# nixorokish/lodestar

Measured on AMD Instinct MI355X. Metric: BLS signature sets verified/sec (1-8 GPUs) + p50 latency @128-set batch, higher is better.
Workload: dtype u32 (381-bit Fp, 12x32-bit Montgomery limbs); 1 GPU; cfg2: 1024 single-pubkey gossip sets per call, batchable requests, random-scalar batch in chunks of 16 requests; each of the 16 contexts submits 22 calls per pass (bls_gpu_verify_many, one device pass, chunks and verdicts per call); sets_per_call=1024, contexts_per_gpu=16, calls_per_pass=22, calls_in_flight_per_gpu=352, parallelism=shard-by-request x1

## Files before the change

### lodestar_amd/build.py

```python
from __future__ import annotations

import concurrent.futures as cf
import hashlib
import json
import os
import re
import subprocess
import sys
from pathlib import Path

ROOT = Path(__file__).resolve().parent.parent
PKG = ROOT / "lodestar_amd"
CSRC = PKG / "csrc"
OUT_DIR = PKG / "_native"
OBJ_DIR = ROOT / "build" / "obj"
LIB = OUT_DIR / "liblodestar_bls.so"
HIPCC = os.environ.get("HIPCC", "/opt/rocm/bin/hipcc")
ARCH = "gfx950"
FLAGS = ["-O3", "-std=c++17", "-fPIC", f"--offload-arch={ARCH}", "-I", str(ROOT / "include"), "-I", str(CSRC)]


def _headers_digest() -> str:
    h = hashlib.sha256()
    for p in sorted(list(CSRC.rglob("*.hpp")) + list((ROOT / "include").glob("*.h"))):
        h.update(p.name.encode())
        h.update(p.read_bytes())
    return h.hexdigest()


def sources() -> list[Path]:
    return [CSRC / "bls_gpu.hip"] + sorted((CSRC / "kernels").glob("*.hip"))


VARIANTS: dict[str, list[str] | dict[str, list[str]]] = {
}


def _variant_flags(variant: str | None, tu: str) -> list[str] | None:
    if not variant:
        return None
    v = VARIANTS[variant]
    return v if isinstance(v, list) else v.get(tu) or None


ADMISSION_BUDGET = 6 << 30
MIN_QUEUES = 4
SIMDS = 1024


def _resources(remarks: str) -> list[dict]:
    out, cur = [], None
    for line in remarks.splitlines():
        if "remark:" not in line:
            continue
        body = line.split("remark:", 1)[1].strip()
        if body.startswith("Function Name:"):
            cur = {"name": body.split(":", 1)[1].strip().split(" ")[0]}
            out.append(cur)
        elif cur is not None and body.startswith("ScratchSize"):
            cur["scratch"] = int(body.split(":", 1)[1].split()[0])
        elif cur is not None and body.startswith("Occupancy"):
            cur["occupancy"] = int(body.split(":", 1)[1].split()[0])
        elif cur is not None and body.startswith("VGPRs:"):
            cur["vgprs"] = int(body.split(":", 1)[1].split()[0])
        elif cur is not None and body.startswith("AGPRs:"):
            cur["agprs"] = int(body.split(":", 1)[1].split()[0])
    for k in out:
        k["device_scratch_bytes"] = k.get("scratch", 0) * 64 * k.get("occupancy", 1) * SIMDS
    return out


def _check_scratch(src: Path, kernels: list[dict]) -> None:
    cap = ADMISSION_BUDGET // MIN_QUEUES
    for k in kernels:
        if k["device_scratch_bytes"] > cap:
            raise SystemExit(f"{src.name}: kernel {k['name']} reserves {k['device_scratch_bytes'] >> 20} MiB of "
                             f"scratch per queue ({k.get('scratch')} B/lane x 64 x {k.get('occupancy')} waves/SIMD "
                             f"x {SIMDS} SIMDs) > {cap >> 20} MiB: fewer than {MIN_QUEUES} contexts would fit the "
                             "runtime's ~8 GiB (lodestar_amd/build.py ADMISSION_BUDGET)")


FIXTURE_TUS = ("k_sign", "k_probe", "k_peak", "k_selftest", "k_selftest_d28")
FIXTURE_KERNELS = ("k_coop_probe", "k_coop_run_test")


def _plain_name(mangled: str) -> str:
    m = re.match(r"_Z(\d+)", mangled)
    return mangled[m.end(): m.end() + int(m.group(1))] if m else mangled


def scratch_per_queue(table: list[dict]) -> tuple[int, str]:
    path = [k for k in table if k.get("tu") not in FIXTURE_TUS and _plain_name(k["name"]) not in FIXTURE_KERNELS]
    worst = max(path, key=lambda k: k["device_scratch_bytes"])
    fixtures = [k for k in table if k not in path]
    deepest = max(fixtures, key=lambda k: k["device_scratch_bytes"], default=None)
    if deepest is not None and deepest["device_scratch_bytes"] > worst["device_scratch_bytes"]:
        raise RuntimeError(
            f"fixture kernel {_plain_name(deepest['name'])} reserves {deepest['device_scratch_bytes']} B of scratch per "
            f"queue, more than the verify path's deepest ({_plain_name(worst['name'])}, "
            f"{worst['device_scratch_bytes']} B): the admission figure would under-count; shrink it or count it")
    return worst["device_scratch_bytes"], _plain_name(worst["name"])


def _compile(src: Path, hdr: str, verbose: bool, extra: list[str] | None = None) -> Path:
    flags = FLAGS + (extra or [])
    key = hashlib.sha256((hdr + " ".join(flags)).encode() + src.read_bytes()).hexdigest()[:16]
    obj = OBJ_DIR / f"{src.stem}.{key}.o"
    res = obj.with_suffix(".res.json")
    if obj.exists() and res.exists():
        return obj
    cmd = [HIPCC, *flags, "-Rpass-analysis=kernel-resource-usage", "-c", str(src), "-o", str(obj) + ".tmp"]
    if verbose:
        print("[build]", " ".join(cmd), flush=True)
    p = subprocess.run(cmd, capture_output=True, text=True)
    if p.returncode != 0:
        sys.stderr.write(p.stderr)
        raise subprocess.CalledProcessError(p.returncode, cmd)
    kernels = _resources(p.stderr)
    _check_scratch(src, kernels)
    res.write_text(json.dumps(kernels, indent=1))
    os.replace(str(obj) + ".tmp", obj)
    return obj


def build_coop_tables(verbose: bool = True) -> Path:
    tools = ROOT / "tools"
    out = OUT_DIR / "coop_tables.bin"
    gz = OUT_DIR / "coop_tables.bin.gz"
    key = hashlib.sha256(b"".join((tools / f).read_bytes()
                                  for f in ("gen_coop.py", "gen_pset.py", "circuits.py", "gen_constants.py"))).hexdigest()
    stamp = OUT_DIR / ".coop_stamp"
    if gz.exists() and out.with_name("coop_programs.json").exists() and stamp.exists() and stamp.read_text() == key:
        return gz
    if not (out.exists() and stamp.exists() and stamp.read_text() == key):
        if verbose:
            print("[build] tools/gen_coop.py ->", out, flush=True)
        subprocess.run([sys.executable, str(tools / "gen_coop.py"), str(out)], check=True)
    import gzip

    with open(out, "rb") as src, gzip.open(str(gz) + ".tmp", "wb", compresslevel=6) as dst:
        dst.write(src.read())
    os.replace(str(gz) + ".tmp", gz)
    stamp.write_text(key)
    return gz


def build_work_model(verbose: bool = True) -> Path:
    out = OUT_DIR / "work_model.json"
    key = hashlib.sha256(_headers_digest().encode() + (ROOT / "tools" / "work_model.cpp").read_bytes()).hexdigest()
    stamp = OUT_DIR / ".work_stamp"
    if out.exists() and stamp.exists() and stamp.read_text() == key:
        return out
    sys.path.insert(0, str(ROOT / "tools"))
    import work_model

    work_model.build(out, verbose)
    stamp.write_text(key)
    return out


def build(jobs: int | None = None, verbose: bool = True, variant: str | None = None) -> Path:
    OUT_DIR.mkdir(parents=True, exist_ok=True)
    OBJ_DIR.mkdir(parents=True, exist_ok=True)
    build_coop_tables(verbose)
    build_work_model(verbose)
    hdr = _headers_digest()
    srcs = sources()
    lib = OUT_DIR / f"liblodestar_bls_{variant}.so" if variant else LIB
    jobs = jobs or min(len(srcs), os.cpu_count() or 4)
    kern_srcs, host_src = srcs[1:], srcs[0]
    with cf.ThreadPoolExecutor(max_workers=jobs) as ex:
        kobjs = list(ex.map(lambda s: _compile(s, hdr, verbose, _variant_flags(variant, s.stem)), kern_srcs))
    table = [dict(k, tu=o.stem.split(".")[0]) for o in kobjs for k in json.loads(o.with_suffix(".res.json").read_text())]
    per_queue, worst = scratch_per_queue(table)
    host_extra = (_variant_flags(variant, host_src.stem) or []) + [f"-DBLS_SCRATCH_PER_QUEUE={per_queue}ull",
                                                                  f'-DBLS_SCRATCH_WORST_KERNEL="{worst}"']
    objs = [_compile(host_src, hdr, verbose, host_extra)] + kobjs
    if not variant:
        (OUT_DIR / "kernel_resources.json").write_text(json.dumps(
            {"scratch_per_queue": per_queue, "scratch_worst_kernel": worst, "kernels": table}, indent=1))
    stamp = hashlib.sha256("".join(str(o) for o in objs).encode()).hexdigest()
    stamp_file = OUT_DIR / (f".lib_stamp_{variant}" if variant else ".lib_stamp")
    if lib.exists() and stamp_file.exists() and stamp_file.read_text() == stamp:
        return lib
    cmd = [HIPCC, f"--offload-arch={ARCH}", "-shared", "-fPIC", "-o", str(lib) + ".tmp", *map(str, objs), "-lz"]
    if verbose:
        print("[build]", " ".join(cmd), flush=True)
    subprocess.run(cmd, check=True)
    os.replace(str(lib) + ".tmp", lib)
    stamp_file.write_text(stamp)
    return lib


def build_hostsim(verbose: bool = True) -> Path:
    src = ROOT / "tests" / "native" / "hostsim.cpp"
    out = ROOT / "tests" / "native" / "libhostsim.so"
    hdr = _headers_digest()
    key = hashlib.sha256(hdr.encode() + src.read_bytes()).hexdigest()[:16]
    stamp = out.with_suffix(".stamp")
    if out.exists() and stamp.exists() and stamp.read_text() == key:
        return out
    cmd = ["g++", "-O2", "-std=c++17", "-shared", "-fPIC", "-DBLS_COUNT_OPS", "-I", str(CSRC), "-I",
           str(ROOT / "include"), "-o", str(out), str(src)]
    if verbose:
        print("[build]", " ".join(cmd), flush=True)
    subprocess.run(cmd, check=True)
    stamp.write_text(key)
    return out


def build_smsum_host(verbose: bool = True, out: Path | None = None, extra: list[str] | None = None) -> Path:
    src = ROOT / "tests" / "native" / "smsum_host.cpp"
    out = out or ROOT / "tests" / "native" / "smsum_host"
    key = hashlib.sha256((_headers_digest() + " ".join(extra or [])).encode() + src.read_bytes()).hexdigest()[:16]
    stamp = out.with_suffix(".stamp")
    if out.exists() and stamp.exists() and stamp.read_text() == key:
        return out
    cmd = ["g++", "-O2", "-std=c++17", *(extra or []), "-I", str(CSRC), "-I", str(ROOT / "include"), "-o", str(out),
           str(src)]
    if verbose:
        print("[build]", " ".join(cmd), flush=True)
    subprocess.run(cmd, check=True)
    stamp.write_text(key)
    return out


def build_cpu_baseline(verbose: bool = True) -> Path:
    out = ROOT / "oracle" / "cpu" / "libbls_cpu.so"
    cmd = ["make", "-s", "-C", str(ROOT / "oracle" / "cpu")]
    if verbose:
        print("[build]", " ".join(cmd), flush=True)
    subprocess.run(cmd, check=True)
    return out


def build_napi(verbose: bool = True) -> Path | None:
    hdr_dir = Path("/usr/include/node")
    if not (hdr_dir / "node_api.h").exists():
        return None
    src = ROOT / "integration" / "napi" / "lodestar_bls_napi.c"
    out = OUT_DIR / "lodestar_bls.node"
    key = hashlib.sha256(src.read_bytes() + (ROOT / "include" / "lodestar_bls.h").read_bytes()).hexdigest()[:16]
    stamp = OUT_DIR / ".napi_stamp"
    if out.exists() and stamp.exists() and stamp.read_text() == key:
        return out
    cmd = ["gcc", "-O2", "-shared", "-fPIC", "-I", str(hdr_dir), "-I", str(ROOT / "include"), str(src),
           "-L", str(OUT_DIR), "-llodestar_bls", "-Wl,-rpath,$ORIGIN", "-o", str(out)]
    if verbose:
        print("[build]", " ".join(cmd), flush=True)
    subprocess.run(cmd, check=True)
    stamp.write_text(key)
    return out


if __name__ == "__main__":
    if len(sys.argv) > 2 and sys.argv[1] == "--variant":
        build(variant=sys.argv[2])
        sys.exit(0)
    build(jobs=int(sys.argv[1]) if len(sys.argv) > 1 else None)
    build_napi()
    build_hostsim()
    build_smsum_host()
    build_cpu_baseline()
```

### lodestar_amd/csrc/bls/field.hpp

```cpp
#pragma once

#include <stdint.h>
#include <string.h>

#if defined(__HIPCC__)
#include <hip/hip_runtime.h>
#define BLS_HD __host__ __device__ __forceinline__
#define BLS_NOINLINE static __host__ __device__ __attribute__((noinline))
#else
#define BLS_HD static inline
#define BLS_NOINLINE static __attribute__((noinline))
#endif

#if defined(BLS_COUNT_OPS) && !defined(__HIP_DEVICE_COMPILE__)
extern unsigned long long bls_fpm_counter;
#define BLS_COUNT_FPM() (++bls_fpm_counter)
#else
#define BLS_COUNT_FPM() ((void)0)
#endif

namespace bls {

struct Fp {
  uint32_t l[12];
};
struct Fp2 {
  Fp c0, c1;
};
struct Fp6 {
  Fp2 c0, c1, c2;
};
struct Fp12 {
  Fp6 c0, c1;
};

}

#include "constants.hpp"

namespace bls {

BLS_HD uint32_t p_limb(int i) {
  const uint32_t t[12] = {BLS_P_LIMBS};
  return t[i];
}

#if defined(__clang__)
BLS_HD uint32_t addc32(uint32_t a, uint32_t b, uint32_t cin, uint32_t* cout) {
  unsigned co;
  unsigned r = __builtin_addc(a, b, cin, &co);
  *cout = co;
  return r;
}
BLS_HD uint32_t subc32(uint32_t a, uint32_t b, uint32_t bin, uint32_t* bout) {
  unsigned bo;
  unsigned r = __builtin_subc(a, b, bin, &bo);
  *bout = bo;
  return r;
}
#else
BLS_HD uint32_t addc32(uint32_t a, uint32_t b, uint32_t cin, uint32_t* cout) {
  uint64_t t = (uint64_t)a + b + cin;
  *cout = (uint32_t)(t >> 32);
  return (uint32_t)t;
}
BLS_HD uint32_t subc32(uint32_t a, uint32_t b, uint32_t bin, uint32_t* bout) {
  uint64_t t = (uint64_t)a - b - bin;
  *bout = (uint32_t)(t >> 63);
  return (uint32_t)t;
}
#endif

BLS_HD Fp fp_zero() {
  Fp r;
#pragma unroll
  for (int i = 0; i < 12; ++i) r.l[i] = 0;
  return r;
}

BLS_HD bool fp_is_zero(const Fp& a) {
  uint32_t acc = 0;
#pragma unroll
  for (int i = 0; i < 12; ++i) acc |= a.l[i];
  return acc == 0;
}

BLS_HD bool fp_eq(const Fp& a, const Fp& b) {
  uint32_t acc = 0;
#pragma unroll
  for (int i = 0; i < 12; ++i) acc |= a.l[i] ^ b.l[i];
  return acc == 0;
}

BLS_HD Fp fp_select(bool c, const Fp& a, const Fp& b) {
  Fp r;
#pragma unroll
  for (int i = 0; i < 12; ++i) r.l[i] = c ? a.l[i] : b.l[i];
  return r;
}

BLS_HD uint32_t fp_sub_p(const Fp& a, Fp& d) {
  uint32_t borrow = 0;
#pragma unroll
  for (int i = 0; i < 12; ++i) d.l[i] = subc32(a.l[i], p_limb(i), borrow, &borrow);
  return borrow;
}

#if defined(__HIPCC__)
}
#include "carry_asm.hpp"
namespace bls {
#endif

#if defined(__HIP_DEVICE_COMPILE__)
BLS_HD Fp fp_reduce_once(const Fp& s) {
  const uint32_t pl[12] = {BLS_P_LIMBS};
  Fp r;
  asm_reduce12(r.l, s.l, pl);
  return r;
}

BLS_HD Fp fp_add(const Fp& a, const Fp& b) {
  Fp s;
  asm_add12(s.l, a.l, b.l);
  return fp_reduce_once(s);
}

BLS_HD Fp fp_sub(const Fp& a, const Fp& b) {
  const uint32_t pl[12] = {BLS_P_LIMBS};
  Fp d, r;
  uint32_t borrow = asm_sub12(d.l, a.l, b.l);
  asm_add12_masked(r.l, d.l, pl, 0u - borrow);
  return r;
}

BLS_HD Fp fp_add_nr(const Fp& a, const Fp& b) {
  Fp s;
  asm_add12(s.l, a.l, b.l);
  return s;
}

BLS_HD Fp fp_sub_nr(const Fp& a, const Fp& b) {
  const uint32_t pl[12] = {BLS_P_LIMBS};
  Fp t, r;
  (void)asm_sub12(t.l, pl, b.l);
  asm_add12(r.l, a.l, t.l);
  return r;
}

BLS_HD Fp fp_reduce_2p(const Fp& a) {
  const uint32_t pl2[12] = {BLS_2P_LIMBS};
  Fp r;
  asm_reduce12(r.l, a.l, pl2);
  return r;
}
#else
static_assert(sizeof(Fp) == 48, "Fp is 6 x 64-bit words on the host");
static inline void fp_w_load(const Fp& a, uint64_t w[6]) { memcpy(w, a.l, 48); }
static inline Fp fp_w_store(const uint64_t w[6]) {
  Fp r;
  memcpy(r.l, w, 48);
  return r;
}
static const uint64_t BLS_P64[6] = {0xb9feffffffffaaabull, 0x1eabfffeb153ffffull, 0x6730d2a0f6b0f624ull,
                                    0x64774b84f38512bfull, 0x4b1ba7b6434bacd7ull, 0x1a0111ea397fe69aull};
#define BLS_NP0_64 0x89f3fffcfffcfffdull

static inline void fp_w_reduce(uint64_t s[6]) {
  uint64_t d[6];
  unsigned __int128 br = 0;
  for (int i = 0; i < 6; ++i) {
    const unsigned __int128 t = (unsigned __int128)s[i] - BLS_P64[i] - (uint64_t)br;
    d[i] = (uint64_t)t;
    br = (t >> 64) & 1;
  }
  if (!br) memcpy(s, d, 48);
}

BLS_HD Fp fp_reduce_once(const Fp& a) {
  uint64_t s[6];
  fp_w_load(a, s);
  fp_w_reduce(s);
  return fp_w_store(s);
}

BLS_HD Fp fp_add(const Fp& a, const Fp& b) {
  uint64_t x[6], y[6];
  fp_w_load(a, x);
  fp_w_load(b, y);
  unsigned __int128 c = 0;
  for (int i = 0; i < 6; ++i) {
    c += (unsigned __int128)x[i] + y[i];
    x[i] = (uint64_t)c;
    c >>= 64;
  }
  fp_w_reduce(x);
  return fp_w_store(x);
}

BLS_HD Fp fp_sub(const Fp& a, const Fp& b) {
  uint64_t x[6], y[6];
  fp_w_load(a, x);
  fp_w_load(b, y);
  unsigned __int128 br = 0;
  for (int i = 0; i < 6; ++i) {
    const unsigned __int128 t = (unsigned __int128)x[i] - y[i] - (uint64_t)br;
    x[i] = (uint64_t)t;
    br = (t >> 64) & 1;
  }
  if (br) {
    unsigned __int128 c = 0;
    for (int i = 0; i < 6; ++i) {
      c += (unsigned __int128)x[i] + BLS_P64[i];
      x[i] = (uint64_t)c;
      c >>= 64;
    }
  }
  return fp_w_store(x);
}

BLS_HD Fp fp_add_nr(const Fp& a, const Fp& b) {
  uint64_t x[6], y[6];
  fp_w_load(a, x);
  fp_w_load(b, y);
  unsigned __int128 c = 0;
  for (int i = 0; i < 6; ++i) {
    c += (unsigned __int128)x[i] + y[i];
    x[i] = (uint64_t)c;
    c >>= 64;
  }
  return fp_w_store(x);
}

BLS_HD Fp fp_sub_nr(const Fp& a, const Fp& b) {
  uint64_t x[6], y[6];
  fp_w_load(a, x);
  fp_w_load(b, y);
  unsigned __int128 br = 0, c = 0;
  for (int i = 0; i < 6; ++i) {
    const unsigned __int128 t = (unsigned __int128)BLS_P64[i] - y[i] - (uint64_t)br;
    y[i] = (uint64_t)t;
    br = (t >> 64) & 1;
  }
  for (int i = 0; i < 6; ++i) {
    c += (unsigned __int128)x[i] + y[i];
    x[i] = (uint64_t)c;
    c >>= 64;
  }
  return fp_w_store(x);
}

BLS_HD Fp fp_reduce_2p(const Fp& a) {
  static const uint64_t P2[6] = {0x73fdffffffff5556ull, 0x3d57fffd62a7ffffull, 0xce61a541ed61ec48ull,
                                 0xc8ee9709e70a257eull, 0x96374f6c869759aeull, 0x340223d472ffcd34ull};
  uint64_t x[6], d[6];
  fp_w_load(a, x);
  unsigned __int128 br = 0;
  for (int i = 0; i < 6; ++i) {
    const unsigned __int128 t = (unsigned __int128)x[i] - P2[i] - (uint64_t)br;
    d[i] = (uint64_t)t;
    br = (t >> 64) & 1;
  }
  return fp_w_store(br ? x : d);
}
#endif

BLS_HD Fp fp_dbl(const Fp& a) { return fp_add(a, a); }

BLS_HD Fp fp_neg(const Fp& a) {
  Fp z = fp_zero();
  return fp_sub(z, a);
}

BLS_HD Fp fp_half(const Fp& a) {
  uint32_t mask = 0u - (a.l[0] & 1u);
  Fp s;
  uint32_t c = 0;
#pragma unroll
  for (int i = 0; i < 12; ++i) s.l[i] = addc32(a.l[i], p_limb(i) & mask, c, &c);
  Fp r;
#pragma unroll
  for (int i = 0; i < 11; ++i) r.l[i] = (s.l[i] >> 1) | (s.l[i + 1] << 31);
  r.l[11] = s.l[11] >> 1;
  return r;
}

#define BLS_D28_MASK 0xFFFFFFFu
#define BLS_NP28 0xFFCFFFDu
BLS_HD uint32_t p28_digit(int k) {
  const uint32_t t[14] = {0xfffaaabu, 0xfefffffu, 0x3ffffb9u, 0xfffeb15u, 0x6241eabu, 0xa0f6b0fu, 0xf6730d2u,
                          0xf38512bu, 0x4774b84u, 0x4bacd76u, 0xba7b643u, 0xe69a4b1u, 0x1ea397fu, 0x001a011u};
  return t[k];
}

BLS_HD void fp_to_d28(const Fp& a, uint32_t d[14]) {
#pragma unroll
  for (int k = 0; k < 14; ++k) {
    const int o = 28 * k, w = o >> 5, s = o & 31;
    const uint64_t pair = ((uint64_t)(w + 1 < 12 ? a.l[w + 1] : 0u) << 32) | a.l[w];
    d[k] = (uint32_t)(pair >> s) & BLS_D28_MASK;
  }
}

#if defined(__HIP_DEVICE_COMPILE__)
#define BLS_D28_MAC(t, a, b)                                                        \
  do {                                                                              \
    uint64_t cc_;                                                                   \
    asm volatile("v_mad_u64_u32 %0, %1, %2, %3, %0" : "+v"(t), "=&s"(cc_) : "v"(a), "v"(b)); \
  } while (0)
#define BLS_D28_MACS(t, a, b)                                                       \
  do {                                                                              \
    uint64_t cc_;                                                                   \
    asm volatile("v_mad_i64_i32 %0, %1, %2, %3, %0" : "+v"(t), "=&s"(cc_) : "v"(a), "v"(b)); \
  } while (0)
#define BLS_PIN_FP(c)                                                                                \
  asm volatile("" ::"v"((c).l[0]), "v"((c).l[1]), "v"((c).l[2]), "v"((c).l[3]), "v"((c).l[4]),     \
               "v"((c).l[5]), "v"((c).l[6]), "v"((c).l[7]), "v"((c).l[8]), "v"((c).l[9]), "v"((c).l[10]), \
               "v"((c).l[11]))
#define BLS_D28_MACK(t, a, k)                                                                        \
  do {                                                                                               \
    uint64_t cc_;                                                                                    \
    asm volatile("v_mad_u64_u32 %0, %1, %2, %3, %0" : "+v"(t), "=&s"(cc_) : "v"(a), "s"(k));        \
  } while (0)
#else
#define BLS_D28_MACK(t, a, k) ((t) += (uint64_t)(a) * (k))
#define BLS_PIN_FP(c) ((void)0)
#define BLS_D28_MAC(t, a, b) ((t) += (uint64_t)(a) * (b))
#define BLS_D28_MACS(t, a, b) ((t) = (uint64_t)((int64_t)(t) + (int64_t)(int32_t)(a) * (int64_t)(int32_t)(b)))
#endif

BLS_HD Fp fp_d28_tail(uint64_t t[27]);

template <bool ORDERED = false>
BLS_HD Fp fp_redc_d28(uint64_t t[27]) {
#pragma unroll
  for (int i = 0; i < 13; ++i) {
    const uint32_t m = ((uint32_t)t[i] * BLS_NP28) & BLS_D28_MASK;
#pragma unroll
    for (int j = 0; j < 14; ++j) {
      if (ORDERED) BLS_D28_MACK(t[i + j], m, p28_digit(j));
      else t[i + j] += (uint64_t)m * p28_digit(j);
    }
    t[i + 1] += t[i] >> 28;
  }
  {
    const uint32_t m = ((uint32_t)t[13] * BLS_NP28) & 0xFFFFFu;
#pragma unroll
    for (int j = 0; j < 14; ++j) {
      if (ORDERED) BLS_D28_MACK(t[13 + j], m, p28_digit(j));
      else t[13 + j] += (uint64_t)m * p28_digit(j);
    }
  }
  return fp_d28_tail(t);
}

BLS_HD Fp fp_d28_tail(uint64_t t[27]) {
  const uint64_t u = t[13] >> 20;
  t[14] += u >> 8;
#pragma unroll
  for (int k = 14; k < 26; ++k) {
    t[k + 1] += t[k] >> 28;
    t[k] &= BLS_D28_MASK;
  }
  Fp r;
  uint64_t acc = u & 0xFFu;
  int nb = 8, w = 0;
#pragma unroll
  for (int k = 14; k < 27; ++k) {
    acc |= t[k] << nb;
    nb += 28;
    while (nb >= 32 && w < 12) {
      r.l[w++] = (uint32_t)acc;
      acc >>= 32;
      nb -= 32;
    }
  }
  while (w < 12) {
    r.l[w++] = (uint32_t)acc;
    acc >>= 32;
  }
  return r;
}

BLS_HD Fp fp_mul_d28_lazy(const Fp& a, const Fp& b) {
  uint32_t x[14], y[14];
  fp_to_d28(a, x);
  fp_to_d28(b, y);
  uint64_t t[27];
#pragma unroll
  for (int k = 0; k < 27; ++k) t[k] = 0;
#pragma unroll
  for (int i = 0; i < 14; ++i)
#pragma unroll
    for (int j = 0; j < 14; ++j) t[i + j] += (uint64_t)x[i] * y[j];
  return fp_redc_d28(t);
}

BLS_HD Fp fp_sqr_d28_lazy(const Fp& a) {
  uint32_t x[14], x2[14];
  fp_to_d28(a, x);
#pragma unroll
  for (int k = 0; k < 14; ++k) x2[k] = x[k] << 1;
  uint64_t t[27];
#pragma unroll
  for (int k = 0; k < 27; ++k) t[k] = 0;
#pragma unroll
  for (int i = 0; i < 14; ++i) {
    t[2 * i] += (uint64_t)x[i] * x[i];
#pragma unroll
    for (int j = i + 1; j < 14; ++j) t[i + j] += (uint64_t)x2[i] * x[j];
  }
  return fp_redc_d28(t);
}

BLS_HD uint64_t c2_col(int k) {
  const uint64_t t[27] = {
      0x00ffffffe1cc48ddull, 0x01ffffffcec8d82dull, 0x02ffffffa9e42d7cull, 0x03ffffff8c5f88ffull, 0x04ffffff683c5c79ull,
      0x05ffffff4a84a061ull, 0x06ffffff2f404920ull, 0x07ffffff0efefe3bull, 0x08fffffee90b358cull, 0x09fffffec66cc7e1ull,
      0x0afffffea7af04abull, 0x0bfffffe892c9c2eull, 0x0cfffffe6149107bull, 0x0c0034009ffe581bull, 0x0b003400bffcbfe9ull,
      0x0a003400dffcbfe8ull, 0x09003400fffcbfe7ull, 0x080034011ffcbfe6ull, 0x070034013ffcbfe5ull, 0x060034015ffcbfe4ull,
      0x050034017ffcbfe3ull, 0x040034019ffcbfe2ull, 0x03003401bffcbfe1ull, 0x02003401dffcbfe0ull, 0x01003401fffcbfdfull,
      0x000034021ffcbfdeull, 0x00000002a4374121ull};
  return t[k];
}

#if defined(__HIP_DEVICE_COMPILE__)
#define BLS_SCHED_FENCE() __builtin_amdgcn_sched_barrier(0)
#else
#define BLS_SCHED_FENCE() ((void)0)
#endif

BLS_HD Fp2 fp2_mul_d28(const Fp& a0, const Fp& a1, const Fp& b0, const Fp& b1) {
  uint32_t x0[14], x1[14], y0[14], y1[14];
  fp_to_d28(a0, x0);
  fp_to_d28(a1, x1);
  fp_to_d28(b0, y0);
  fp_to_d28(b1, y1);
  uint64_t t[27];
  int32_t ny1[14];
#pragma unroll
  for (int j = 0; j < 14; ++j) ny1[j] = -(int32_t)y1[j];
#pragma unroll
  for (int k = 0; k < 27; ++k) t[k] = c2_col(k);
#pragma unroll
  for (int i = 0; i < 14; ++i)
#pragma unroll
    for (int j = 0; j < 14; ++j) {
      BLS_D28_MAC(t[i + j], x0[i], y0[j]);
      BLS_D28_MACS(t[i + j], x1[i], ny1[j]);
    }
  const Fp c0 = fp_reduce_once(fp_redc_d28<true>(t));
  BLS_PIN_FP(c0);
  BLS_SCHED_FENCE();
#pragma unroll
  for (int k = 0; k < 27; ++k) t[k] = 0;
#pragma unroll
  for (int i = 0; i < 14; ++i)
#pragma unroll
    for (int j = 0; j < 14; ++j) {
      BLS_D28_MAC(t[i + j], x0[i], y1[j]);
      BLS_D28_MAC(t[i + j], x1[i], y0[j]);
    }
  return Fp2{c0, fp_reduce_once(fp_redc_d28<true>(t))};
}

BLS_HD Fp2 fp2_sqr_d28(const Fp& a0, const Fp& a1) {
  uint32_t x0[14], x1[14];
  fp_to_d28(a0, x0);
  fp_to_d28(a1, x1);
  uint64_t t[27];
  int32_t n1[14], n2[14];
#pragma unroll
  for (int j = 0; j < 14; ++j) {
    n1[j] = -(int32_t)x1[j];
    n2[j] = -(int32_t)(x1[j] << 1);
  }
#pragma unroll
  for (int k = 0; k < 27; ++k) t[k] = c2_col(k);
#pragma unroll
  for (int i = 0; i < 14; ++i) {
    BLS_D28_MAC(t[2 * i], x0[i], x0[i]);
    BLS_D28_MACS(t[2 * i], x1[i], n1[i]);
#pragma unroll
    for (int j = i + 1; j < 14; ++j) {
      BLS_D28_MAC(t[i + j], x0[i] << 1, x0[j]);
      BLS_D28_MACS(t[i + j], x1[i], n2[j]);
    }
  }
  const Fp c0 = fp_reduce_once(fp_redc_d28<true>(t));
  BLS_PIN_FP(c0);
  BLS_SCHED_FENCE();
#pragma unroll
  for (int k = 0; k < 27; ++k) t[k] = 0;
#pragma unroll
  for (int i = 0; i < 14; ++i)
#pragma unroll
    for (int j = 0; j < 14; ++j) BLS_D28_MAC(t[i + j], x0[i] << 1, x1[j]);
  return Fp2{c0, fp_reduce_once(fp_redc_d28<true>(t))};
}

#if defined(__HIP_DEVICE_COMPILE__)
__device__ __forceinline__ void bls_mac(uint64_t& lo, uint32_t& hi, uint32_t a, uint32_t b) {
  uint64_t cc;
  asm("v_mad_u64_u32 %0, %2, %3, %4, %0\n\t"
      "v_addc_co_u32 %1, %2, 0, %1, %2"
      : "+v"(lo), "+v"(hi), "=&s"(cc)
      : "v"(a), "v"(b));
}
__device__ __forceinline__ void bls_mac_s(uint64_t& lo, uint32_t& hi, uint32_t a, uint32_t b) {
  uint64_t cc;
  asm("v_mad_u64_u32 %0, %2, %3, %4, %0\n\t"
      "v_addc_co_u32 %1, %2, 0, %1, %2"
      : "+v"(lo), "+v"(hi), "=&s"(cc)
      : "v"(a), "s"(b));
}
__device__ __forceinline__ void bls_mac2(uint64_t& lo, uint32_t& hi, uint32_t a, uint32_t b, uint64_t& lo2,
                                         uint32_t& hi2, uint32_t m, uint32_t p) {
  uint64_t c1, c2;
  asm("v_mad_u64_u32 %0, %4, %6, %7, %0\n\t"
      "v_mad_u64_u32 %2, %5, %8, %9, %2\n\t"
      "v_addc_co_u32 %1, %4, 0, %1, %4\n\t"
      "v_addc_co_u32 %3, %5, 0, %3, %5"
      : "+v"(lo), "+v"(hi), "+v"(lo2), "+v"(hi2), "=&s"(c1), "=&s"(c2)
      : "v"(a), "v"(b), "v"(m), "s"(p));
}

#define BLS_MAC4(L, H, k, x, y0, y1, y2, y3, YC)                                                       \
  do {                                                                                             \
    uint64_t c0_, c1_, c2_, c3_;                                                                   \
    asm("v_mad_u64_u32 %0, %8, %12, %13, %0\n\t"                                                  \
        "v_mad_u64_u32 %2, %9, %12, %14, %2\n\t"                                                  \
        "v_mad_u64_u32 %4, %10, %12, %15, %4\n\t"                                                 \
        "v_mad_u64_u32 %6, %11, %12, %16, %6\n\t"                                                 \
        "v_addc_co_u32 %1, %8, 0, %1, %8\n\t"                                                     \
        "v_addc_co_u32 %3, %9, 0, %3, %9\n\t"                                                     \
        "v_addc_co_u32 %5, %10, 0, %5, %10\n\t"                                                   \
        "v_addc_co_u32 %7, %11, 0, %7, %11"                                                        \
        : "+v"(L[k]), "+v"(H[k]), "+v"(L[k + 1]), "+v"(H[k + 1]), "+v"(L[k + 2]), "+v"(H[k + 2]),   \
          "+v"(L[k + 3]), "+v"(H[k + 3]), "=&s"(c0_), "=&s"(c1_), "=&s"(c2_), "=&s"(c3_)            \
        : "v"(x), YC(y0), YC(y1), YC(y2), YC(y3));                                                  \
  } while (0)

__device__ __forceinline__ void bls_col_add(uint64_t& lo, uint32_t& hi, uint64_t c) {
  uint32_t l0 = (uint32_t)lo, l1 = (uint32_t)(lo >> 32);
  uint64_t cc;
  asm("v_add_co_u32 %0, %3, %0, %4\n\t"
      "v_addc_co_u32 %1, %3, %1, %5, %3\n\t"
      "v_addc_co_u32 %2, %3, 0, %2, %3"
      : "+v"(l0), "+v"(l1), "+v"(hi), "=&s"(cc)
      : "v"((uint32_t)c), "v"((uint32_t)(c >> 32)));
  lo = ((uint64_t)l1 << 32) | l0;
}

template <bool LAZY>
__device__ __forceinline__ Fp fp_mul_cols(const Fp& a, const Fp& b) {
  uint64_t L[24];
  uint32_t H[24];
#pragma unroll
  for (int k = 0; k < 24; ++k) {
    L[k] = 0;
    H[k] = 0;
  }
#pragma unroll
  for (int i = 0; i < 12; ++i) {
#pragma unroll
    for (int j = 0; j < 12; j += 4) BLS_MAC4(L, H, i + j, a.l[i], b.l[j], b.l[j + 1], b.l[j + 2], b.l[j + 3], "v");
  }
#pragma unroll
  for (int i = 0; i < 12; ++i) {
    const uint32_t m = (uint32_t)L[i] * BLS_NP0;
    BLS_MAC4(L, H, i, m, p_limb(0), p_limb(1), p_limb(2), p_limb(3), "s");
    const uint64_t c = (L[i] >> 32) | ((uint64_t)H[i] << 32);
    bls_col_add(L[i + 1], H[i + 1], c);
    BLS_MAC4(L, H, i + 4, m, p_limb(4), p_limb(5), p_limb(6), p_limb(7), "s");
    BLS_MAC4(L, H, i + 8, m, p_limb(8), p_limb(9), p_limb(10), p_limb(11), "s");
  }
  Fp u;
#pragma unroll
  for (int k = 12; k < 23; ++k) {
    u.l[k - 12] = (uint32_t)L[k];
    const uint64_t c = (L[k] >> 32) | ((uint64_t)H[k] << 32);
    bls_col_add(L[k + 1], H[k + 1], c);
  }
  u.l[11] = (uint32_t)L[23];
  return LAZY ? u : fp_reduce_once(u);
}
__device__ __forceinline__ Fp fp_sqr_cols(const Fp& a) {
  uint64_t L[24];
  uint32_t H[24];
#pragma unroll
  for (int k = 0; k < 24; ++k) {
    L[k] = 0;
    H[k] = 0;
  }
#pragma unroll
  for (int i = 0; i < 11; ++i) {
    int j = i + 1;
#pragma unroll
    for (; j + 3 < 12; j += 4) BLS_MAC4(L, H, i + j, a.l[i], a.l[j], a.l[j + 1], a.l[j + 2], a.l[j + 3], "v");
#pragma unroll
    for (; j < 12; ++j) bls_mac(L[i + j], H[i + j], a.l[i], a.l[j]);
  }
#pragma unroll
  for (int k = 1; k < 23; ++k) {
    H[k] = (H[k] << 1) | (uint32_t)(L[k] >> 63);
    L[k] <<= 1;
  }
#pragma unroll
  for (int i = 0; i < 12; ++i) bls_mac(L[2 * i], H[2 * i], a.l[i], a.l[i]);
#pragma unroll
  for (int i = 0; i < 12; ++i) {
    const uint32_t m = (uint32_t)L[i] * BLS_NP0;
    BLS_MAC4(L, H, i, m, p_limb(0), p_limb(1), p_limb(2), p_limb(3), "s");
    const uint64_t c = (L[i] >> 32) | ((uint64_t)H[i] << 32);
    bls_col_add(L[i + 1], H[i + 1], c);
    BLS_MAC4(L, H, i + 4, m, p_limb(4), p_limb(5), p_limb(6), p_limb(7), "s");
    BLS_MAC4(L, H, i + 8, m, p_limb(8), p_limb(9), p_limb(10), p_limb(11), "s");
  }
  Fp u;
#pragma unroll
  for (int k = 12; k < 23; ++k) {
    u.l[k - 12] = (uint32_t)L[k];
    const uint64_t c = (L[k] >> 32) | ((uint64_t)H[k] << 32);
    bls_col_add(L[k + 1], H[k + 1], c);
  }
  u.l[11] = (uint32_t)L[23];
  return fp_reduce_once(u);
}
#ifdef BLS_FP_INLINE
#define BLS_FP_MUL_ATTR static __device__ __forceinline__
#else
#define BLS_FP_MUL_ATTR BLS_NOINLINE
#endif
#if !defined(BLS_FP_D28)
BLS_FP_MUL_ATTR Fp fp_sqr_dev(Fp a) { return fp_sqr_cols(a); }
__device__ __forceinline__ Fp fp_mul_inl(const Fp& a, const Fp& b) { return fp_mul_cols<false>(a, b); }
__device__ __forceinline__ Fp fp_mul_lazy(const Fp& a, const Fp& b) { return fp_mul_cols<true>(a, b); }
#else
BLS_FP_MUL_ATTR Fp fp_sqr_dev(Fp a) { return fp_reduce_once(fp_sqr_d28_lazy(a)); }
__device__ __forceinline__ Fp fp_mul_inl(const Fp& a, const Fp& b) { return fp_reduce_once(fp_mul_d28_lazy(a, b)); }
__device__ __forceinline__ Fp fp_mul_lazy(const Fp& a, const Fp& b) { return fp_mul_d28_lazy(a, b); }
#endif
#define BLS_W12(x) uint32_t x##0, uint32_t x##1, uint32_t x##2, uint32_t x##3, uint32_t x##4, uint32_t x##5, \
                   uint32_t x##6, uint32_t x##7, uint32_t x##8, uint32_t x##9, uint32_t x##10, uint32_t x##11
#define BLS_FP_OF(x) Fp{{x##0, x##1, x##2, x##3, x##4, x##5, x##6, x##7, x##8, x##9, x##10, x##11}}
#define BLS_L12(v) (v).l[0], (v).l[1], (v).l[2], (v).l[3], (v).l[4], (v).l[5], (v).l[6], (v).l[7], (v).l[8], \
                   (v).l[9], (v).l[10], (v).l[11]
BLS_FP_MUL_ATTR Fp fp_mul_w(BLS_W12(a), BLS_W12(b)) { return fp_mul_inl(BLS_FP_OF(a), BLS_FP_OF(b)); }
BLS_FP_MUL_ATTR Fp fp_sqr_w(BLS_W12(a)) { return fp_sqr_dev(BLS_FP_OF(a)); }
__device__ __forceinline__ Fp fp_mul(const Fp& a, const Fp& b) { return fp_mul_w(BLS_L12(a), BLS_L12(b)); }
#else
BLS_HD Fp fp_mul(const Fp& a, const Fp& b) {
  BLS_COUNT_FPM();
  typedef unsigned __int128 u128;
  uint64_t x[6], y[6], t[13];
  fp_w_load(a, x);
  fp_w_load(b, y);
  for (int k = 0; k < 13; ++k) t[k] = 0;
  for (int i = 0; i < 6; ++i) {
    uint64_t c = 0;
    for (int j = 0; j < 6; ++j) {
      const u128 v = (u128)x[i] * y[j] + t[i + j] + c;
      t[i + j] = (uint64_t)v;
      c = (uint64_t)(v >> 64);
    }
    t[i + 6] = c;
  }
  for (int i = 0; i < 6; ++i) {
    const uint64_t m = t[i] * BLS_NP0_64;
    uint64_t c = 0;
    for (int j = 0; j < 6; ++j) {
      const u128 v = (u128)m * BLS_P64[j] + t[i + j] + c;
      t[i + j] = (uint64_t)v;
      c = (uint64_t)(v >> 64);
    }
    for (int k = i + 6; k < 13 && c; ++k) {
      const u128 v = (u128)t[k] + c;
      t[k] = (uint64_t)v;
      c = (uint64_t)(v >> 64);
    }
  }
  fp_w_reduce(t + 6);
  return fp_w_store(t + 6);
}
BLS_HD Fp fp_mul_inl(const Fp& a, const Fp& b) { return fp_mul(a, b); }
BLS_HD Fp fp_mul_lazy(const Fp& a, const Fp& b) { return fp_mul(a, b); }
#endif

#if defined(__HIP_DEVICE_COMPILE__)
BLS_HD Fp fp_sqr(const Fp& a) { return fp_sqr_w(BLS_L12(a)); }
#else
BLS_HD Fp fp_sqr(const Fp& a) { return fp_mul(a, a); }
#endif

BLS_HD Fp fp_to_mont(const Fp& a) { return fp_mul(a, c_r2()); }

BLS_HD Fp fp_from_mont(const Fp& a) {
  Fp one = fp_zero();
  one.l[0] = 1;
  return fp_mul(a, one);
}

}
#include "lazy28.hpp"
namespace bls {

#if defined(__HIP_DEVICE_COMPILE__) && !defined(BLS_LAZY_POW)
#define BLS_LAZY_POW 1
#endif
#ifdef BLS_LAZY_POW
template <uint32_t (*E)(int), int BITS>
BLS_HD Fp fp_pow_const(const Fp& a) {
  return lz_pow_const<E, BITS>(a);
}
#else
template <uint32_t (*E)(int), int BITS>
BLS_HD Fp fp_pow_const(const Fp& a) {
  Fp tab[8];
  tab[0] = a;
  const Fp a2 = fp_sqr(a);
  for (int k = 1; k < 8; ++k) tab[k] = fp_mul(tab[k - 1], a2);
  Fp r = a;
  bool started = false;
  int i = BITS - 1;
  while (i >= 0) {
    if (!((E(i >> 5) >> (i & 31)) & 1u)) {
      r = fp_sqr(r);
      --i;
      continue;
    }
    int j = i - 3 < 0 ? 0 : i - 3;
    while (!((E(j >> 5) >> (j & 31)) & 1u)) ++j;
    uint32_t val = 0;
    for (int k = i; k >= j; --k) {
      val = (val << 1) | ((E(k >> 5) >> (k & 31)) & 1u);
      if (started) r = fp_sqr(r);
    }
    r = started ? fp_mul(r, tab[val >> 1]) : tab[val >> 1];
    started = true;
    i = j - 1;
  }
  return r;
}
#endif

BLS_HD Fp fp_inv(const Fp& a) { return fp_pow_const<e_p_minus_2, E_P_MINUS_2_BITS>(a); }

BLS_HD bool big_is_one(const Fp& a) {
  uint32_t acc = a.l[0] ^ 1u;
#pragma unroll
  for (int i = 1; i < 12; ++i) acc |= a.l[i];
  return acc == 0;
}

BLS_HD void big_shr1(Fp& a) {
#pragma unroll
  for (int i = 0; i < 11; ++i) a.l[i] = (a.l[i] >> 1) | (a.l[i + 1] << 31);
  a.l[11] >>= 1;
}

BLS_HD bool big_geq(const Fp& a, const Fp& b) {
  uint32_t borrow = 0;
#pragma unroll
  for (int i = 0; i < 12; ++i) {
    uint64_t t = (uint64_t)a.l[i] - b.l[i] - borrow;
    borrow = (uint32_t)(t >> 63);
  }
  return borrow == 0;
}

BLS_HD void big_sub(Fp& a, const Fp& b) {
  uint32_t borrow = 0;
#pragma unroll
  for (int i = 0; i < 12; ++i) {
    uint64_t t = (uint64_t)a.l[i] - b.l[i] - borrow;
    a.l[i] = (uint32_t)t;
    borrow = (uint32_t)(t >> 63);
  }
}

struct Big13 {
  uint32_t l[13];
};

BLS_HD Big13 big13_lin_shr30(const Big13& x, const Big13& y, int32_t u, int32_t v) {
  uint32_t t[13];
  int64_t carry = 0;
#pragma unroll
  for (int i = 0; i < 13; ++i) {
    const int64_t xi = i < 12 ? (int64_t)x.l[i] : (int64_t)(int32_t)x.l[i];
    const int64_t yi = i < 12 ? (int64_t)y.l[i] : (int64_t)(int32_t)y.l[i];
    const int64_t s = carry + (int64_t)u * xi + (int64_t)v * yi;
    t[i] = (uint32_t)s;
    carry = s >> 32;
  }
  Big13 r;
#pragma unroll
  for (int i = 0; i < 12; ++i) r.l[i] = (t[i] >> 30) | (t[i + 1] << 2);
  r.l[12] = (uint32_t)((int32_t)t[12] >> 30);
  return r;
}

BLS_HD Big13 big13_lin_modp_shr30(const Big13& d, const Big13& e, int32_t u, int32_t v) {
  uint32_t t[13];
  int64_t carry = 0;
#pragma unroll
  for (int i = 0; i < 13; ++i) {
    const int64_t di = i < 12 ? (int64_t)d.l[i] : (int64_t)(int32_t)d.l[i];
    const int64_t ei = i < 12 ? (int64_t)e.l[i] : (int64_t)(int32_t)e.l[i];
    const int64_t s = carry + (int64_t)u * di + (int64_t)v * ei;
    t[i] = (uint32_t)s;
    carry = s >> 32;
  }
  const uint32_t k = (t[0] * BLS_NP0) & 0x3fffffffu;
  uint64_t c = 0;
#pragma unroll
  for (int i = 0; i < 12; ++i) {
    const uint64_t s = (uint64_t)t[i] + (uint64_t)k * p_limb(i) + c;
    t[i] = (uint32_t)s;
    c = s >> 32;
  }
  t[12] += (uint32_t)c;
  Big13 r;
#pragma unroll
  for (int i = 0; i < 12; ++i) r.l[i] = (t[i] >> 30) | (t[i + 1] << 2);
  r.l[12] = (uint32_t)((int32_t)t[12] >> 30);
  Big13 m;
  uint32_t borrow = 0;
#pragma unroll
  for (int i = 0; i < 13; ++i) {
    const uint64_t s = (uint64_t)r.l[i] - (i < 12 ? p_limb(i) : 0u) - borrow;
    m.l[i] = (uint32_t)s;
    borrow = (uint32_t)(s >> 63);
  }
  const bool ge_p = (int32_t)m.l[12] >= 0;
  uint32_t cc = 0;
  Big13 q;
#pragma unroll
  for (int i = 0; i < 13; ++i) {
    const uint64_t s = (uint64_t)r.l[i] + (i < 12 ? p_limb(i) : 0u) + cc;
    q.l[i] = (uint32_t)s;
    cc = (uint32_t)(s >> 32);
  }
  const bool lt_mp = (int32_t)q.l[12] < 0;
#pragma unroll
  for (int i = 0; i < 13; ++i) r.l[i] = ge_p ? m.l[i] : (lt_mp ? q.l[i] : r.l[i]);
  return r;
}

BLS_NOINLINE Fp fp_inv_gcd(Fp a) {
  if (fp_is_zero(a)) return fp_zero();
  Big13 f, g, d, e;
#pragma unroll
  for (int i = 0; i < 12; ++i) {
    f.l[i] = p_limb(i);
    g.l[i] = a.l[i];
    d.l[i] = 0;
    e.l[i] = 0;
  }
  f.l[12] = g.l[12] = d.l[12] = e.l[12] = 0;
  e.l[0] = 1;
  int32_t delta = 1;
  for (int round = 0; round < 37; ++round) {
    uint32_t fl = f.l[0], gl = g.l[0];
    int32_t u = 1, v = 0, q = 0, r = 1;
    for (int s = 0; s < 30; ++s) {
      const bool godd = (gl & 1u) != 0;
      const bool swap = godd && delta > 0;
      const uint32_t nfl = swap ? gl : fl, ngl = swap ? (0u - fl) : gl;
      const int32_t nu = swap ? q : u, nv = swap ? r : v, nq = swap ? -u : q, nr = swap ? -v : r;
      delta = swap ? -delta : delta;
      fl = nfl;
      gl = ngl;
      u = nu;
      v = nv;
      q = nq;
      r = nr;
      gl += godd ? fl : 0u;
      q += godd ? u : 0;
      r += godd ? v : 0;
      gl >>= 1;
      u *= 2;
      v *= 2;
      delta += 1;
    }
    const Big13 f2 = big13_lin_shr30(f, g, u, v);
    const Big13 g2 = big13_lin_shr30(f, g, q, r);
    const Big13 d2 = big13_lin_modp_shr30(d, e, u, v);
    const Big13 e2 = big13_lin_modp_shr30(d, e, q, r);
    f = f2;
    g = g2;
    d = d2;
    e = e2;
  }
  const bool fneg = (int32_t)f.l[12] < 0;
  Big13 x;
  uint32_t borrow = 0;
#pragma unroll
  for (int i = 0; i < 13; ++i) {
    const uint64_t s = (uint64_t)0 - d.l[i] - borrow;
    x.l[i] = fneg ? (uint32_t)s : d.l[i];
    borrow = (uint32_t)(s >> 63);
  }
  const bool xneg = (int32_t)x.l[12] < 0;
  Fp inv;
  uint32_t c = 0;
#pragma unroll
  for (int i = 0; i < 12; ++i) {
    const uint64_t s = (uint64_t)x.l[i] + (xneg ? p_limb(i) : 0u) + c;
    inv.l[i] = (uint32_t)s;
    c = (uint32_t)(s >> 32);
  }
  return fp_mul(inv, c_r3());
}


BLS_HD bool fp_plain_gt_half(const Fp& a) {
  const uint32_t h[12] = {BLS_HALF_P_LIMBS};
  uint32_t borrow = 0;
#pragma unroll
  for (int i = 0; i < 12; ++i) {
    uint64_t t = (uint64_t)h[i] - a.l[i] - borrow;
    borrow = (uint32_t)(t >> 63);
  }
  return borrow != 0;
}

BLS_HD bool fp_lex_largest(const Fp& a_mont) { return fp_plain_gt_half(fp_from_mont(a_mont)); }

BLS_HD bool fp_plain_is_canonical(const Fp& a) {
  Fp d;
  return fp_sub_p(a, d) != 0;
}

BLS_HD Fp fp_from_be48(const uint8_t* b) {
  Fp r;
#pragma unroll
  for (int k = 0; k < 12; ++k) {
    const uint8_t* q = b + 44 - 4 * k;
    r.l[k] = ((uint32_t)q[0] << 24) | ((uint32_t)q[1] << 16) | ((uint32_t)q[2] << 8) | (uint32_t)q[3];
  }
  return r;
}

BLS_HD void fp_to_be48(const Fp& a, uint8_t* b) {
#pragma unroll
  for (int k = 0; k < 12; ++k) {
    uint8_t* q = b + 44 - 4 * k;
    q[0] = (uint8_t)(a.l[k] >> 24);
    q[1] = (uint8_t)(a.l[k] >> 16);
    q[2] = (uint8_t)(a.l[k] >> 8);
    q[3] = (uint8_t)a.l[k];
  }
}

BLS_HD bool fp_sqrt(const Fp& a, Fp& r) {
  r = fp_pow_const<e_p_plus_1_div_4, E_P_PLUS_1_DIV_4_BITS>(a);
  return fp_eq(fp_sqr(r), a);
}

BLS_HD Fp2 fp2_zero() { return Fp2{fp_zero(), fp_zero()}; }
BLS_HD Fp2 fp2_one() { return Fp2{c_one(), fp_zero()}; }
BLS_HD bool fp2_is_zero(const Fp2& a) { return fp_is_zero(a.c0) && fp_is_zero(a.c1); }
BLS_HD bool fp2_eq(const Fp2& a, const Fp2& b) { return fp_eq(a.c0, b.c0) && fp_eq(a.c1, b.c1); }
BLS_HD Fp2 fp2_select(bool c, const Fp2& a, const Fp2& b) {
  return Fp2{fp_select(c, a.c0, b.c0), fp_select(c, a.c1, b.c1)};
}
BLS_HD Fp2 fp2_add(const Fp2& a, const Fp2& b) { return Fp2{fp_add(a.c0, b.c0), fp_add(a.c1, b.c1)}; }
BLS_HD Fp2 fp2_sub(const Fp2& a, const Fp2& b) { return Fp2{fp_sub(a.c0, b.c0), fp_sub(a.c1, b.c1)}; }
BLS_HD Fp2 fp2_dbl(const Fp2& a) { return Fp2{fp_dbl(a.c0), fp_dbl(a.c1)}; }
BLS_HD Fp2 fp2_neg(const Fp2& a) { return Fp2{fp_neg(a.c0), fp_neg(a.c1)}; }
BLS_HD Fp2 fp2_conj(const Fp2& a) { return Fp2{a.c0, fp_neg(a.c1)}; }
BLS_HD Fp2 fp2_half(const Fp2& a) { return Fp2{fp_half(a.c0), fp_half(a.c1)}; }
BLS_HD Fp2 fp2_mul_fp(const Fp2& a, const Fp& b) { return Fp2{fp_mul(a.c0, b), fp_mul(a.c1, b)}; }

BLS_HD Fp2 fp2_mul(const Fp2& a, const Fp2& b) {
  Fp t0 = fp_mul(a.c0, b.c0);
  Fp t1 = fp_mul(a.c1, b.c1);
  Fp t2 = fp_mul(fp_add_nr(a.c0, a.c1), fp_add_nr(b.c0, b.c1));
  return Fp2{fp_sub(t0, t1), fp_sub(fp_sub(t2, t0), t1)};
}

BLS_HD Fp2 fp2_mul_s(const Fp2& a, const Fp2& b) {
  Fp t0 = fp_mul(a.c0, b.c0);
  Fp t1 = fp_mul(a.c1, b.c1);
  Fp t2 = fp_mul(fp_reduce_2p(fp_add_nr(a.c0, a.c1)), fp_add_nr(b.c0, b.c1));
  return Fp2{fp_sub(t0, t1), fp_sub(fp_sub(t2, t0), t1)};
}
BLS_HD Fp2 fp2_add_nr(const Fp2& a, const Fp2& b) { return Fp2{fp_add_nr(a.c0, b.c0), fp_add_nr(a.c1, b.c1)}; }

BLS_HD Fp2 fp2_sqr(const Fp2& a) {
  Fp t0 = fp_mul(fp_add_nr(a.c0, a.c1), fp_sub_nr(a.c0, a.c1));
  Fp t1 = fp_mul(fp_add_nr(a.c0, a.c0), a.c1);
  return Fp2{t0, t1};
}

BLS_HD Fp2 fp2_mul_xi(const Fp2& a) { return Fp2{fp_sub(a.c0, a.c1), fp_add(a.c0, a.c1)}; }

BLS_HD Fp2 fp2_inv(const Fp2& a) {
  Fp n = fp_add(fp_sqr(a.c0), fp_sqr(a.c1));
  Fp ni = fp_inv(n);
  return Fp2{fp_mul(a.c0, ni), fp_neg(fp_mul(a.c1, ni))};
}

BLS_HD uint32_t fp2_sgn0(const Fp2& a) {
  Fp p0 = fp_from_mont(a.c0);
  Fp p1 = fp_from_mont(a.c1);
  uint32_t s0 = p0.l[0] & 1u;
  uint32_t z0 = fp_is_zero(p0) ? 1u : 0u;
  uint32_t s1 = p1.l[0] & 1u;
  return s0 | (z0 & s1);
}

BLS_HD bool fp2_lex_largest(const Fp2& a) {
  Fp p1 = fp_from_mont(a.c1);
  if (!fp_is_zero(p1)) return fp_plain_gt_half(p1);
  return fp_plain_gt_half(fp_from_mont(a.c0));
}

BLS_HD bool fp2_sqrt(const Fp2& a, Fp2& r) {
  if (fp_is_zero(a.c1)) {
    Fp s;
    if (fp_sqrt(a.c0, s)) {
      r = Fp2{s, fp_zero()};
      return true;
    }
    fp_sqrt(fp_neg(a.c0), s);
    r = Fp2{fp_zero(), s};
    return true;
  }
  Fp alpha = fp_add(fp_sqr(a.c0), fp_sqr(a.c1));
  Fp gamma;
  if (!fp_sqrt(alpha, gamma)) return false;
  Fp d = fp_half(fp_add(a.c0, gamma));
  Fp t = fp_pow_const<e_p_minus_3_div_4, E_P_MINUS_3_DIV_4_BITS>(d);
  Fp dt = fp_mul(d, t);
  Fp a1t2 = fp_half(fp_mul(a.c1, t));
  if (fp_eq(fp_sqr(dt), d)) {
    r = Fp2{dt, a1t2};
  } else {
    r = Fp2{a1t2, fp_neg(dt)};
  }
  return true;
}

BLS_HD Fp6 fp6_zero() { return Fp6{fp2_zero(), fp2_zero(), fp2_zero()}; }
BLS_HD Fp6 fp6_one() { return Fp6{fp2_one(), fp2_zero(), fp2_zero()}; }
BLS_HD Fp6 fp6_add(const Fp6& a, const Fp6& b) {
  return Fp6{fp2_add(a.c0, b.c0), fp2_add(a.c1, b.c1), fp2_add(a.c2, b.c2)};
}
BLS_HD Fp6 fp6_sub(const Fp6& a, const Fp6& b) {
  return Fp6{fp2_sub(a.c0, b.c0), fp2_sub(a.c1, b.c1), fp2_sub(a.c2, b.c2)};
}
BLS_HD Fp6 fp6_neg(const Fp6& a) { return Fp6{fp2_neg(a.c0), fp2_neg(a.c1), fp2_neg(a.c2)}; }
BLS_HD bool fp6_eq(const Fp6& a, const Fp6& b) {
  return fp2_eq(a.c0, b.c0) && fp2_eq(a.c1, b.c1) && fp2_eq(a.c2, b.c2);
}
BLS_HD Fp6 fp6_mul_v(const Fp6& a) { return Fp6{fp2_mul_xi(a.c2), a.c0, a.c1}; }

BLS_HD Fp6 fp6_mul(const Fp6& a, const Fp6& b) {
  Fp2 t0 = fp2_mul(a.c0, b.c0);
  Fp2 t1 = fp2_mul(a.c1, b.c1);
  Fp2 t2 = fp2_mul(a.c2, b.c2);
  Fp2 c0 = fp2_sub(fp2_sub(fp2_mul_s(fp2_add_nr(a.c1, a.c2), fp2_add_nr(b.c1, b.c2)), t1), t2);
  c0 = fp2_add(fp2_mul_xi(c0), t0);
  Fp2 c1 = fp2_sub(fp2_sub(fp2_mul_s(fp2_add_nr(a.c0, a.c1), fp2_add_nr(b.c0, b.c1)), t0), t1);
  c1 = fp2_add(c1, fp2_mul_xi(t2));
  Fp2 c2 = fp2_sub(fp2_sub(fp2_mul_s(fp2_add_nr(a.c0, a.c2), fp2_add_nr(b.c0, b.c2)), t0), t2);
  c2 = fp2_add(c2, t1);
  return Fp6{c0, c1, c2};
}

BLS_HD Fp6 fp6_sqr(const Fp6& a) { return fp6_mul(a, a); }

BLS_HD Fp6 fp6_mul_01(const Fp6& a, const Fp2& d0, const Fp2& d1) {
  Fp2 a0d0 = fp2_mul(a.c0, d0);
  Fp2 a1d1 = fp2_mul(a.c1, d1);
  Fp2 c0 = fp2_add(a0d0, fp2_mul_xi(fp2_mul(a.c2, d1)));
  Fp2 c1 = fp2_sub(fp2_sub(fp2_mul_s(fp2_add_nr(a.c0, a.c1), fp2_add_nr(d0, d1)), a0d0), a1d1);
  Fp2 c2 = fp2_add(a1d1, fp2_mul(a.c2, d0));
  return Fp6{c0, c1, c2};
}

BLS_HD Fp6 fp6_mul_1(const Fp6& a, const Fp2& d1) {
  return Fp6{fp2_mul_xi(fp2_mul(a.c2, d1)), fp2_mul(a.c0, d1), fp2_mul(a.c1, d1)};
}

BLS_HD Fp6 fp6_inv(const Fp6& a) {
  Fp2 t0 = fp2_sub(fp2_sqr(a.c0), fp2_mul_xi(fp2_mul(a.c1, a.c2)));
  Fp2 t1 = fp2_sub(fp2_mul_xi(fp2_sqr(a.c2)), fp2_mul(a.c0, a.c1));
  Fp2 t2 = fp2_sub(fp2_sqr(a.c1), fp2_mul(a.c0, a.c2));
  Fp2 n = fp2_add(fp2_mul(a.c0, t0), fp2_mul_xi(fp2_add(fp2_mul(a.c2, t1), fp2_mul(a.c1, t2))));
  Fp2 ni = fp2_inv(n);
  return Fp6{fp2_mul(t0, ni), fp2_mul(t1, ni), fp2_mul(t2, ni)};
}

BLS_HD Fp12 fp12_one() { return Fp12{fp6_one(), fp6_zero()}; }
BLS_HD bool fp12_eq(const Fp12& a, const Fp12& b) { return fp6_eq(a.c0, b.c0) && fp6_eq(a.c1, b.c1); }
BLS_HD bool fp12_is_one(const Fp12& a) { return fp12_eq(a, fp12_one()); }
BLS_HD Fp12 fp12_conj(const Fp12& a) { return Fp12{a.c0, fp6_neg(a.c1)}; }

BLS_NOINLINE Fp12 fp12_mul(const Fp12& a, const Fp12& b) {
  Fp6 t0 = fp6_mul(a.c0, b.c0);
  Fp6 t1 = fp6_mul(a.c1, b.c1);
  Fp6 c1 = fp6_sub(fp6_sub(fp6_mul(fp6_add(a.c0, a.c1), fp6_add(b.c0, b.c1)), t0), t1);
  Fp6 c0 = fp6_add(t0, fp6_mul_v(t1));
  return Fp12{c0, c1};
}

BLS_NOINLINE Fp12 fp12_sqr(const Fp12& a) {
  Fp6 ab = fp6_mul(a.c0, a.c1);
  Fp6 s = fp6_mul(fp6_add(a.c0, a.c1), fp6_add(a.c0, fp6_mul_v(a.c1)));
  Fp6 c0 = fp6_sub(fp6_sub(s, ab), fp6_mul_v(ab));
  Fp6 c1 = fp6_add(ab, ab);
  return Fp12{c0, c1};
}

BLS_NOINLINE Fp12 fp12_mul_line(const Fp12& f, const Fp2& l0, const Fp2& l2, const Fp2& l3) {
  Fp6 aa = fp6_mul_01(f.c0, l0, l2);
  Fp6 bb = fp6_mul_1(f.c1, l3);
  Fp6 c1 = fp6_sub(fp6_sub(fp6_mul_01(fp6_add(f.c0, f.c1), l0, fp2_add(l2, l3)), aa), bb);
  Fp6 c0 = fp6_add(aa, fp6_mul_v(bb));
  return Fp12{c0, c1};
}

BLS_HD Fp12 fp12_mul_line2(const Fp12& f, const Fp2& l0, const Fp2& l2, const Fp2& l3, const Fp2& m0,
                           const Fp2& m2, const Fp2& m3) {
  const Fp2 m00 = fp2_mul(l0, m0), m22 = fp2_mul(l2, m2), m33 = fp2_mul(l3, m3);
  const Fp2 a0 = fp2_add(m00, fp2_mul_xi(m33));
  const Fp2 a2 = fp2_sub(fp2_sub(fp2_mul_s(fp2_add_nr(l0, l2), fp2_add_nr(m0, m2)), m00), m22);
  const Fp2 a3 = fp2_sub(fp2_sub(fp2_mul_s(fp2_add_nr(l0, l3), fp2_add_nr(m0, m3)), m00), m33);
  const Fp2 a5 = fp2_sub(fp2_sub(fp2_mul_s(fp2_add_nr(l2, l3), fp2_add_nr(m2, m3)), m22), m33);
  const Fp6 p0 = Fp6{a0, a2, m22};
  const Fp6 t0 = fp6_mul(f.c0, p0);
  const Fp6 t1 = fp6_mul_v(fp6_mul_01(f.c1, a3, a5));
  const Fp6 c1 = fp6_sub(fp6_sub(fp6_mul(fp6_add(f.c0, f.c1), Fp6{a0, fp2_add(a2, a3), fp2_add(m22, a5)}), t0), t1);
  return Fp12{fp6_add(t0, fp6_mul_v(t1)), c1};
}

BLS_HD Fp6 fp12_sqr_half_prod(const Fp12& a, bool h) {
  return fp6_mul(h ? fp6_add(a.c0, a.c1) : a.c0, h ? fp6_add(a.c0, fp6_mul_v(a.c1)) : a.c1);
}
BLS_HD Fp12 fp12_sqr_half_join(const Fp6& own, const Fp6& other, bool h) {
  const Fp6 ab = h ? other : own, s = h ? own : other;
  return Fp12{fp6_sub(fp6_sub(s, ab), fp6_mul_v(ab)), fp6_add(ab, ab)};
}
struct LineHalf {
  Fp6 m;
  Fp2 p, q;
};
BLS_HD LineHalf fp12_line_half_prod(const Fp12& f, const Fp2& l0, const Fp2& l2, const Fp2& l3, bool h) {
  LineHalf r;
  r.m = fp6_mul_01(h ? fp6_add(f.c0, f.c1) : f.c0, l0, h ? fp2_add(l2, l3) : l2);
  r.p = fp2_mul(h ? f.c1.c0 : f.c1.c2, l3);
  r.q = fp2_mul(f.c1.c1, l3);
  return r;
}
BLS_HD Fp12 fp12_line_half_join(const LineHalf& own, const Fp6& m_other, const Fp2& p_other, bool h) {
  const Fp6 aa = h ? m_other : own.m, t = h ? own.m : m_other;
  const Fp6 bb = Fp6{fp2_mul_xi(h ? p_other : own.p), h ? own.p : p_other, own.q};
  return Fp12{fp6_add(aa, fp6_mul_v(bb)), fp6_sub(fp6_sub(t, aa), bb)};
}

BLS_HD Fp12 fp12_inv(const Fp12& a) {
  Fp6 n = fp6_sub(fp6_sqr(a.c0), fp6_mul_v(fp6_sqr(a.c1)));
  Fp6 ni = fp6_inv(n);
  return Fp12{fp6_mul(a.c0, ni), fp6_neg(fp6_mul(a.c1, ni))};
}

BLS_HD Fp12 fp12_frob(const Fp12& a) {
  Fp12 r;
  r.c0.c0 = fp2_conj(a.c0.c0);
  r.c1.c0 = fp2_mul(fp2_conj(a.c1.c0), c_frob1_1());
  r.c0.c1 = fp2_mul(fp2_conj(a.c0.c1), c_frob1_2());
  r.c1.c1 = fp2_mul(fp2_conj(a.c1.c1), c_frob1_3());
  r.c0.c2 = fp2_mul(fp2_conj(a.c0.c2), c_frob1_4());
  r.c1.c2 = fp2_mul(fp2_conj(a.c1.c2), c_frob1_5());
  return r;
}

BLS_HD Fp12 fp12_frob2(const Fp12& a) {
  Fp12 r;
  r.c0.c0 = a.c0.c0;
  r.c1.c0 = fp2_mul_fp(a.c1.c0, c_frob2_1());
  r.c0.c1 = fp2_mul_fp(a.c0.c1, c_frob2_2());
  r.c1.c1 = fp2_mul_fp(a.c1.c1, c_frob2_3());
  r.c0.c2 = fp2_mul_fp(a.c0.c2, c_frob2_4());
  r.c1.c2 = fp2_mul_fp(a.c1.c2, c_frob2_5());
  return r;
}

BLS_HD void fp4_sqr(const Fp2& x, const Fp2& y, Fp2& rx, Fp2& ry) {
  Fp2 t0 = fp2_sqr(x);
  Fp2 t1 = fp2_sqr(y);
  rx = fp2_add(t0, fp2_mul_xi(t1));
  ry = fp2_sub(fp2_sub(fp2_sqr(fp2_add(x, y)), t0), t1);
}

BLS_NOINLINE Fp12 fp12_cyclotomic_sqr(const Fp12& f) {
  Fp2 a0, a1, b0, b1, d0, d1;
  fp4_sqr(f.c0.c0, f.c1.c1, a0, a1);
  fp4_sqr(f.c1.c0, f.c0.c2, b0, b1);
  fp4_sqr(f.c0.c1, f.c1.c2, d0, d1);
  Fp12 r;
  r.c0.c0 = fp2_add(fp2_dbl(fp2_sub(a0, f.c0.c0)), a0);
  r.c1.c1 = fp2_add(fp2_dbl(fp2_add(a1, f.c1.c1)), a1);
  Fp2 xd1 = fp2_mul_xi(d1);
  r.c1.c0 = fp2_add(fp2_dbl(fp2_add(xd1, f.c1.c0)), xd1);
  r.c0.c2 = fp2_add(fp2_dbl(fp2_sub(d0, f.c0.c2)), d0);
  r.c0.c1 = fp2_add(fp2_dbl(fp2_sub(b0, f.c0.c1)), b0);
  r.c1.c2 = fp2_add(fp2_dbl(fp2_add(b1, f.c1.c2)), b1);
  return r;
}

}
```

### lodestar_amd/csrc/kernels/field_ops.hpp

```cpp
#pragma once

#include "../launchers.hpp"
#include "../bls/selftest_ops.hpp"

namespace bls {

enum : uint32_t {
  FOP_ADD = 0,
  FOP_SUB,
  FOP_NEG,
  FOP_DBL,
  FOP_HALF,
  FOP_ADD_NR,
  FOP_SUB_NR,
  FOP_REDUCE_ONCE,
  FOP_REDUCE_2P,
  FOP_CANON3,
  FOP_MUL,
  FOP_SQR,
  FOP_MUL_LAZY,
  FOP_SQR_D28_LAZY,
  FOP_FP2_MUL_D28,
  FOP_FP2_SQR_D28,
  FOP_FP2_MUL,
  FOP_FP2_SQR,
  FOP_FP2_MUL_S,
  FOP_LZ_MUL_RAW,
  FOP_LZ_SQR_RAW,
  FOP_LZ_FP_OPS,
  FOP_LZ_FP2_OPS,
  FOP_INV,
  FOP_INV_GCD,
  FOP_SQRT,
  FOP_FP2_INV,
  FOP_FP2_SQRT,
  FOP_LIN8,
  FOP_COUNT
};
#define FOP_D28_FLAG 0x100u
#define FOP_LIN8_IN 102

constexpr int field_op_in_words(uint32_t op) {
  return op == FOP_NEG || op == FOP_DBL || op == FOP_HALF || op == FOP_REDUCE_ONCE || op == FOP_REDUCE_2P ||
                 op == FOP_CANON3 || op == FOP_SQR || op == FOP_SQR_D28_LAZY || op == FOP_INV ||
                 op == FOP_INV_GCD || op == FOP_SQRT
             ? 12
         : op == FOP_FP2_MUL_D28 || op == FOP_FP2_MUL || op == FOP_FP2_MUL_S || op == FOP_LZ_FP2_OPS ? 48
         : op == FOP_LZ_MUL_RAW                                                                        ? 28
         : op == FOP_LZ_SQR_RAW                                                                        ? 14
         : op == FOP_LIN8                                                                              ? FOP_LIN8_IN
                                                                                                       : 24;
}
constexpr int field_op_out_words(uint32_t op) {
  return op == FOP_FP2_MUL_D28 || op == FOP_FP2_SQR_D28 || op == FOP_FP2_MUL || op == FOP_FP2_SQR ||
                 op == FOP_FP2_MUL_S || op == FOP_FP2_INV
             ? 24
         : op == FOP_LZ_MUL_RAW || op == FOP_LZ_SQR_RAW ? 14
         : op == FOP_LZ_FP_OPS                          ? 120
         : op == FOP_LZ_FP2_OPS                         ? 144
         : op == FOP_SQRT                               ? 13
         : op == FOP_FP2_SQRT                           ? 25
                                                        : 12;
}

constexpr bool field_op_d28_only(uint32_t op) { return op == FOP_CANON3 || op >= FOP_SQR_D28_LAZY; }

#if defined(BLS_FP_D28)
#define FOP_IS_D28 true
#else
#define FOP_IS_D28 false
#endif

__device__ __forceinline__ Fp fop_ld(const uint32_t* w, int k) {
  Fp r;
#pragma unroll
  for (int i = 0; i < 12; ++i) r.l[i] = w[12 * k + i];
  return r;
}
__device__ __forceinline__ void fop_st(uint32_t* w, int k, const Fp& v) {
#pragma unroll
  for (int i = 0; i < 12; ++i) w[12 * k + i] = v.l[i];
}
__device__ __forceinline__ Fp2 fop_ld2(const uint32_t* w, int k) { return Fp2{fop_ld(w, 2 * k), fop_ld(w, 2 * k + 1)}; }
__device__ __forceinline__ void fop_st2(uint32_t* w, int k, const Fp2& v) {
  fop_st(w, 2 * k, v.c0);
  fop_st(w, 2 * k + 1, v.c1);
}

template <uint32_t OP, bool D28>
__device__ __forceinline__ void field_op_body(const uint32_t* x, uint32_t* y) {
  if constexpr (OP == FOP_ADD) fop_st(y, 0, fp_add(fop_ld(x, 0), fop_ld(x, 1)));
  else if constexpr (OP == FOP_SUB) fop_st(y, 0, fp_sub(fop_ld(x, 0), fop_ld(x, 1)));
  else if constexpr (OP == FOP_NEG) fop_st(y, 0, fp_neg(fop_ld(x, 0)));
  else if constexpr (OP == FOP_DBL) fop_st(y, 0, fp_dbl(fop_ld(x, 0)));
  else if constexpr (OP == FOP_HALF) fop_st(y, 0, fp_half(fop_ld(x, 0)));
  else if constexpr (OP == FOP_ADD_NR) fop_st(y, 0, fp_add_nr(fop_ld(x, 0), fop_ld(x, 1)));
  else if constexpr (OP == FOP_SUB_NR) fop_st(y, 0, fp_sub_nr(fop_ld(x, 0), fop_ld(x, 1)));
  else if constexpr (OP == FOP_REDUCE_ONCE) fop_st(y, 0, fp_reduce_once(fop_ld(x, 0)));
  else if constexpr (OP == FOP_REDUCE_2P) fop_st(y, 0, fp_reduce_2p(fop_ld(x, 0)));
  else if constexpr (OP == FOP_CANON3) fop_st(y, 0, fp_canon3(fop_ld(x, 0)));
  else if constexpr (OP == FOP_MUL) fop_st(y, 0, fp_mul(fop_ld(x, 0), fop_ld(x, 1)));
  else if constexpr (OP == FOP_SQR) fop_st(y, 0, fp_sqr(fop_ld(x, 0)));
  else if constexpr (OP == FOP_MUL_LAZY) fop_st(y, 0, fp_mul_lazy(fop_ld(x, 0), fop_ld(x, 1)));
#if defined(BLS_FP_D28)
  else if constexpr (OP == FOP_SQR_D28_LAZY) fop_st(y, 0, fp_sqr_d28_lazy(fop_ld(x, 0)));
  else if constexpr (OP == FOP_FP2_MUL_D28)
    fop_st2(y, 0, fp2_mul_d28(fop_ld(x, 0), fop_ld(x, 1), fop_ld(x, 2), fop_ld(x, 3)));
  else if constexpr (OP == FOP_FP2_SQR_D28) fop_st2(y, 0, fp2_sqr_d28(fop_ld(x, 0), fop_ld(x, 1)));
  else if constexpr (OP == FOP_FP2_MUL) fop_st2(y, 0, fp2_mul(fop_ld2(x, 0), fop_ld2(x, 1)));
  else if constexpr (OP == FOP_FP2_SQR) fop_st2(y, 0, fp2_sqr(fop_ld2(x, 0)));
  else if constexpr (OP == FOP_FP2_MUL_S) fop_st2(y, 0, fp2_mul_s(fop_ld2(x, 0), fop_ld2(x, 1)));
  else if constexpr (OP == FOP_LZ_MUL_RAW || OP == FOP_LZ_SQR_RAW) {
    Lz14 a, b;
#pragma unroll
    for (int k = 0; k < 14; ++k) {
      a.d[k] = (int32_t)x[k];
      b.d[k] = OP == FOP_LZ_MUL_RAW ? (int32_t)x[14 + k] : 0;
    }
    const Lz14 r = OP == FOP_LZ_MUL_RAW ? lz_mul_w(LZ_L14(a), LZ_L14(b)) : lz_sqr_w(LZ_L14(a));
#pragma unroll
    for (int k = 0; k < 14; ++k) y[k] = (uint32_t)r.d[k];
  } else if constexpr (OP == FOP_LZ_FP_OPS) {
    Fp r[10];
    sf_lz_fp_ops(fop_ld(x, 0), fop_ld(x, 1), r);
    for (int k = 0; k < 10; ++k) fop_st(y, k, r[k]);
  } else if constexpr (OP == FOP_LZ_FP2_OPS) {
    Fp2 r[6];
    sf_lz_fp2_ops(fop_ld2(x, 0), fop_ld2(x, 1), r);
    for (int k = 0; k < 6; ++k) fop_st2(y, k, r[k]);
  } else if constexpr (OP == FOP_INV) fop_st(y, 0, fp_inv(fop_ld(x, 0)));
  else if constexpr (OP == FOP_INV_GCD) fop_st(y, 0, fp_inv_gcd(fop_ld(x, 0)));
  else if constexpr (OP == FOP_SQRT) {
    Fp r = fp_zero();
    y[0] = fp_sqrt(fop_ld(x, 0), r) ? 1u : 0u;
    fop_st(y + 1, 0, r);
  } else if constexpr (OP == FOP_FP2_INV) fop_st2(y, 0, fp2_inv(fop_ld2(x, 0)));
  else if constexpr (OP == FOP_FP2_SQRT) {
    Fp2 r = fp2_zero();
    y[0] = fp2_sqrt(fop_ld2(x, 0), r) ? 1u : 0u;
    fop_st2(y + 1, 0, r);
  }
#endif
}

template <uint32_t OP, bool D28, int IN, int OUT>
__global__ __launch_bounds__(BLS_BLOCK) void k_field_op(const uint32_t* __restrict__ in, uint32_t n,
                                                        uint32_t* __restrict__ out) {
  const uint32_t i = blockIdx.x * BLS_BLOCK + threadIdx.x;
  if (i >= n) return;
  uint32_t x[IN], y[OUT];
#pragma unroll
  for (int k = 0; k < IN; ++k) x[k] = in[(size_t)IN * i + k];
#pragma unroll
  for (int k = 0; k < OUT; ++k) y[k] = 0;
  field_op_body<OP, D28>(x, y);
#pragma unroll
  for (int k = 0; k < OUT; ++k) out[(size_t)OUT * i + k] = y[k];
}

#if defined(BLS_FP_D28)
template <bool D28>
__global__ __launch_bounds__(BLS_BLOCK) void k_field_lin8(const uint32_t* __restrict__ in, uint32_t n,
                                                          uint32_t* __restrict__ out) {
  __shared__ Fp vals[BLS_BLOCK * 8];
  __shared__ int s_nmax;
  const uint32_t lane = threadIdx.x, i = blockIdx.x * BLS_BLOCK + lane;
  const bool live = i < n;
  if (lane == 0) s_nmax = 0;
  __syncthreads();
  uint16_t refs[8];
  int16_t cf[8];
#pragma unroll
  for (int k = 0; k < 8; ++k) {
    refs[k] = 0;
    cf[k] = 0;
  }
  int nt = 0;
  bool single = false;
  if (live) {
    const uint32_t* rec = in + (size_t)FOP_LIN8_IN * i;
    nt = rec[100] < 8u ? (int)rec[100] : 8;
    single = (rec[101] & 1u) != 0;
#pragma unroll
    for (int k = 0; k < 8; ++k) {
      lds_store_fp(vals, lane * 8 + k, fop_ld(rec, k));
      if (k < nt) {
        refs[k] = (uint16_t)(lane * 8 + k);
        cf[k] = (int16_t)(rec[96 + (k >> 1)] >> (16 * (k & 1)));
      }
    }
    atomicMax(&s_nmax, nt);
  }
  __syncthreads();
  const int nmax = __builtin_amdgcn_readfirstlane(s_nmax);
  const Fp r = coop_lin(refs, cf, nt, nmax, single, (const LdsU4*)vals);
  if (live) fop_st(out + 12ull * i, 0, r);
}
#endif

#define FOP_CASE(OP)                                                                                    \
  case OP:                                                                                              \
    k_field_op<OP, FOP_IS_D28, field_op_in_words(OP), field_op_out_words(OP)>                            \
        <<<bls_grid_for(n), BLS_BLOCK, 0, s>>>(in, n, out);                                             \
    break

static hipError_t field_op_launch(uint32_t op, const uint32_t* in, uint32_t n, uint32_t* out, hipStream_t s) {
  switch (op) {
    FOP_CASE(FOP_ADD);
    FOP_CASE(FOP_SUB);
    FOP_CASE(FOP_NEG);
    FOP_CASE(FOP_DBL);
    FOP_CASE(FOP_HALF);
    FOP_CASE(FOP_ADD_NR);
    FOP_CASE(FOP_SUB_NR);
    FOP_CASE(FOP_REDUCE_ONCE);
    FOP_CASE(FOP_REDUCE_2P);
    FOP_CASE(FOP_MUL);
    FOP_CASE(FOP_SQR);
    FOP_CASE(FOP_MUL_LAZY);
#if defined(BLS_FP_D28)
    FOP_CASE(FOP_CANON3);
    FOP_CASE(FOP_SQR_D28_LAZY);
    FOP_CASE(FOP_FP2_MUL_D28);
    FOP_CASE(FOP_FP2_SQR_D28);
    FOP_CASE(FOP_FP2_MUL);
    FOP_CASE(FOP_FP2_SQR);
    FOP_CASE(FOP_FP2_MUL_S);
    FOP_CASE(FOP_LZ_MUL_RAW);
    FOP_CASE(FOP_LZ_SQR_RAW);
    FOP_CASE(FOP_LZ_FP_OPS);
    FOP_CASE(FOP_LZ_FP2_OPS);
    FOP_CASE(FOP_INV);
    FOP_CASE(FOP_INV_GCD);
    FOP_CASE(FOP_SQRT);
    FOP_CASE(FOP_FP2_INV);
    FOP_CASE(FOP_FP2_SQRT);
    case FOP_LIN8:
      k_field_lin8<true><<<bls_grid_for(n), BLS_BLOCK, 0, s>>>(in, n, out);
      break;
#endif
    default:
      return hipErrorInvalidValue;
  }
  return hipGetLastError();
}

}
```

### lodestar_amd/csrc/kernels/k_chain.hip

```cpp
#define BLS_FP_D28 1
#include "../launchers.hpp"

using namespace bls;

namespace {

__device__ __noinline__ void iso_jac_nl(G2J* out, const Fp* q) { *out = iso_map_jac(Fp2{q[0], q[1]}, Fp2{q[2], q[3]}); }

__device__ __noinline__ void g2_mul_aff(G2J* out, const G2A* in, uint64_t k) { *out = aff_mul_u64(*in, k); }
__device__ __noinline__ void g2_mul_r(G2J* out, const G2A* in, uint64_t k, G2J* T) {
  uint32_t a, b;
  glv_split(k, a, b);
  *out = in->inf ? jac_infinity<Fp2>() : jac_mul_glv<Fp2>(jac_from_aff(*in), a, b, T);
}
__device__ __noinline__ void g1_mul_r(G1J* out, const G1J* in, uint64_t k, G1J* T) {
  uint32_t a, b;
  glv_split(k, a, b);
  *out = jac_mul_glv<Fp>(*in, a, b, T);
}
__device__ __noinline__ void g2_add(G2J* out, const G2J* a, const G2J* b) { *out = jac_add(*a, *b); }

__device__ __noinline__ void g2_to_aff(G2A* out, const G2J* in) {
  if (jac_is_inf(*in)) {
    out->x = fp2_zero();
    out->y = fp2_zero();
    out->inf = true;
    return;
  }
  const Fp ni = fp_inv_gcd(fp_add(fp_sqr(in->z.c0), fp_sqr(in->z.c1)));
  const Fp2 zi = Fp2{fp_mul(in->z.c0, ni), fp_neg(fp_mul(in->z.c1, ni))};
  const Fp2 zi2 = fp2_sqr(zi);
  out->x = fp2_mul(in->x, zi2);
  out->y = fp2_mul(in->y, fp2_mul(zi2, zi));
  out->inf = false;
}

__device__ __noinline__ void g2_mul_x_aff(G2J* out, const G2J* p) {
  G2A a;
  g2_to_aff(&a, p);
  g2_mul_aff(out, &a, (uint64_t)BLS_X_ABS);
  out->y = fp2_neg(out->y);
}

__device__ void store_one(Fp12* f) {
  Fp* d = reinterpret_cast<Fp*>(f);
  d[0] = c_one();
#pragma unroll
  for (int k = 1; k < 12; ++k) d[k] = fp_zero();
}

__device__ void flag_exact(const PipeBufs& b, uint32_t i) {
  b.set_flag[i] = 1u;
  atomicAdd(b.flag_count, 1u);
}

}

__device__ bool chain_skip(const PipeBufs& b, uint32_t i) {
  return b.pk_status[i] != BLS_OK || b.sig_status[i] != BLS_OK || jac_is_inf(b.pk[i]) || b.sig[i].inf ||
         b.set_flag[i];
}

__device__ __noinline__ void chain_role_h(Fp* chain, const Fp* qs, uint8_t* chain_st, uint32_t i) {
  Fp* o = chain + (size_t)CHAIN_WORDS * i;
  const Fp* q = qs + 8ull * i;
  G2J A, B, C;
  iso_jac_nl(&A, q);
  iso_jac_nl(&B, q + 4);
  g2_add(&A, &A, &B);
  g2_mul_x_aff(&B, &A);
  C = g2_psi(A);
  g2_add(&B, &B, &C);
  C = g2_psi(g2_psi(jac_dbl(A)));
  g2_add(&A, &B, &A);
  A.y = fp2_neg(A.y);
  g2_add(&C, &C, &A);
  g2_mul_x_aff(&A, &B);
  g2_add(&A, &A, &C);
  chain_st[4 * i + 0] = jac_is_inf(A) ? 1 : 0;
  if (jac_is_inf(A)) return;
  const Fp ni = fp_inv_gcd(fp_add(fp_sqr(A.z.c0), fp_sqr(A.z.c1)));
  const Fp2 zi = Fp2{fp_mul(A.z.c0, ni), fp_neg(fp_mul(A.z.c1, ni))};
  const Fp2 zi2 = fp2_sqr(zi);
  const Fp2 hx = fp2_mul(A.x, zi2);
  const Fp2 hy = fp2_mul(A.y, fp2_mul(zi2, zi));
  o[CH_HQ + 0] = hx.c0;
  o[CH_HQ + 1] = hx.c1;
  o[CH_HQ + 2] = hy.c0;
  o[CH_HQ + 3] = hy.c1;
}

__device__ __noinline__ void chain_role_sub(const G2A* sigs, uint8_t* chain_st, uint32_t i) {
  const G2A sig = sigs[i];
  G2J xs;
  g2_mul_aff(&xs, &sig, (uint64_t)BLS_X_ABS);
  chain_st[4 * i + 1] = jac_eq(g2_psi(jac_from_aff(sig)), jac_neg(xs)) ? 0 : 1;
}

__device__ __noinline__ void chain_role_rs(Fp* chain, const G2A* sigs, const uint32_t* seed, uint32_t scalar_base,
                                           G2J* rtab2, uint32_t i) {
  Fp* o = chain + (size_t)CHAIN_WORDS * i;
  const G2A sig = sigs[i];
  G2J RS;
  g2_mul_r(&RS, &sig, set_scalar(seed, scalar_base + i), rtab2 + 15ull * i);
  o[CH_RS + 0] = RS.x.c0;
  o[CH_RS + 1] = RS.x.c1;
  o[CH_RS + 2] = RS.y.c0;
  o[CH_RS + 3] = RS.y.c1;
  o[CH_RS + 4] = RS.z.c0;
  o[CH_RS + 5] = RS.z.c1;
}

__device__ __noinline__ void chain_role_rp(Fp* chain, const G1J* pks, uint8_t* chain_st, const uint32_t* seed,
                                           uint32_t scalar_base, G1J* rtab1, uint32_t i) {
  Fp* o = chain + (size_t)CHAIN_WORDS * i;
  G1J RP;
  const G1J pk = pks[i];
  g1_mul_r(&RP, &pk, set_scalar(seed, scalar_base + i), rtab1 + 15ull * i);
  chain_st[4 * i + 3] = jac_is_inf(RP) ? 1 : 0;
  if (jac_is_inf(RP)) return;
  o[CH_RP + 0] = RP.x;
  o[CH_RP + 1] = RP.y;
  o[CH_RP + 2] = RP.z;
}

#define BLS_CHAIN_ATTR __attribute__((amdgpu_waves_per_eu(2)))
__global__ __launch_bounds__(BLS_BLOCK) BLS_CHAIN_ATTR void k_chain(PipeBufs b, uint32_t blocks_per_role,
                                                                   uint32_t roles) {
  uint32_t role = 0, nth = blockIdx.x / blocks_per_role;
  for (uint32_t m = roles;; m &= m - 1) {
    if (nth-- == 0) {
      role = (uint32_t)__builtin_ctz(m);
      break;
    }
  }
  const uint32_t i = (blockIdx.x % blocks_per_role) * BLS_BLOCK + threadIdx.x;
  if (i >= b.n_sets) return;
  if (role == 0 ? ((b.msg_rep && b.msg_rep[i] != i) || b.set_flag[i]) : chain_skip(b, i)) return;
  if (role == 0) chain_role_h(b.chain, b.q, b.chain_st, i);
  else if (role == 1) chain_role_sub(b.sig, b.chain_st, i);
  else if (role == 2) chain_role_rs(b.chain, b.sig, b.seed, b.scalar_base, b.rtab2, i);
  else chain_role_rp(b.chain, b.pk, b.chain_st, b.seed, b.scalar_base, b.rtab1, i);
}

__global__ __launch_bounds__(BLS_BLOCK) void k_chain_done(PipeBufs b) {
  BLS_TAIL_PRIO();
  const uint32_t i = blockIdx.x * BLS_BLOCK + threadIdx.x;
  if (i >= b.n_sets) return;
  b.chain_live[i] = 0u;
  if (b.pk_status[i] != BLS_OK || b.sig_status[i] != BLS_OK || jac_is_inf(b.pk[i])) {
    store_one(&b.f[i]);
    return;
  }
  if (b.sig[i].inf || b.set_flag[i]) {
    flag_exact(b, i);
    return;
  }
  const uint8_t* st = b.chain_st + 4 * i;
  if (st[1]) {
    b.sig_status[i] = BLS_POINT_NOT_IN_GROUP;
    store_one(&b.f[i]);
    return;
  }
  const uint32_t rep = b.msg_rep ? b.msg_rep[i] : i;
  if (b.chain_st[4 * rep + 0] || st[3]) {
    flag_exact(b, i);
    return;
  }
  if (rep != i) {
    const Fp* src = b.chain + (size_t)CHAIN_WORDS * rep + CH_HQ;
    Fp* dst = b.chain + (size_t)CHAIN_WORDS * i + CH_HQ;
#pragma unroll
    for (int k = 0; k < 4; ++k) dst[k] = src[k];
  }
  if (b.set_unit && b.set_unit[i] != UNIT_NONE) store_one(&b.f[i]);
  b.chain_live[i] = 1u;
}

hipError_t launch_k_chain(const PipeBufs& b, hipStream_t s, uint32_t roles) {
  const uint32_t nb = bls_grid_for(b.n_sets);
  roles &= 0xFu;
  if (roles == 0) return hipSuccess;
  k_chain<<<(uint32_t)__builtin_popcount(roles) * nb, BLS_BLOCK, 0, s>>>(b, nb, roles);
  if (roles != 0x4u) k_chain_done<<<nb, BLS_BLOCK, 0, s>>>(b);
  return hipGetLastError();
}
```

### lodestar_amd/csrc/kernels/k_mlq.hip

```cpp
#define BLS_FP_D28 1
#include <stdlib.h>

#include "../launchers.hpp"
#include "bls/pairing.hpp"

using namespace bls;

namespace {

constexpr int ML_EVENTS = 68;
constexpr int LINE_WORDS = 6 * 12;

__device__ __forceinline__ bool ml_live(const PipeBufs& b, uint32_t i, uint32_t units_paired) {
  if (!b.chain_live[i]) return false;
  return !(units_paired && b.set_unit && i < b.n_sets && b.set_unit[i] != UNIT_NONE);
}

__device__ __forceinline__ size_t line_at(uint32_t stride, uint32_t k, int e, int w) {
  return ((size_t)e * LINE_WORDS + w) * stride + k;
}

__device__ __forceinline__ void store_line(uint32_t* L, uint32_t stride, uint32_t k, int e, const G1Eval& P,
                                           const Fp2& c0, const Fp2& c1, const Fp2& c2) {
  const Fp2 l[3] = {c0, fp2_mul_fp(c1, P.xz), fp2_mul_fp(c2, P.y)};
#pragma unroll
  for (int j = 0; j < 3; ++j)
#pragma unroll
    for (int w = 0; w < 12; ++w) {
      L[line_at(stride, k, e, 24 * j + w)] = l[j].c0.l[w];
      L[line_at(stride, k, e, 24 * j + 12 + w)] = l[j].c1.l[w];
    }
}

__device__ __forceinline__ void load_line(const uint32_t* L, uint32_t stride, uint32_t k, int e, Fp2& l0, Fp2& l2,
                                          Fp2& l3) {
  Fp2* l[3] = {&l0, &l2, &l3};
#pragma unroll
  for (int j = 0; j < 3; ++j)
#pragma unroll
    for (int w = 0; w < 12; ++w) {
      l[j]->c0.l[w] = L[line_at(stride, k, e, 24 * j + w)];
      l[j]->c1.l[w] = L[line_at(stride, k, e, 24 * j + 12 + w)];
    }
}

__device__ __forceinline__ Fp12 sqr12(const Fp12& a) {
  const Fp6 ab = fp6_mul(a.c0, a.c1);
  const Fp6 s = fp6_mul(fp6_add(a.c0, a.c1), fp6_add(a.c0, fp6_mul_v(a.c1)));
  return Fp12{fp6_sub(fp6_sub(s, ab), fp6_mul_v(ab)), fp6_add(ab, ab)};
}

__device__ __forceinline__ Fp12 mul_line12(const Fp12& f, const Fp2& l0, const Fp2& l2, const Fp2& l3) {
  const Fp6 aa = fp6_mul_01(f.c0, l0, l2);
  const Fp6 bb = fp6_mul_1(f.c1, l3);
  const Fp6 c1 = fp6_sub(fp6_sub(fp6_mul_01(fp6_add(f.c0, f.c1), l0, fp2_add(l2, l3)), aa), bb);
  return Fp12{fp6_add(aa, fp6_mul_v(bb)), c1};
}

__device__ __forceinline__ Fp12 ml_f(const uint32_t* L, uint32_t stride, uint32_t k0, uint32_t n) {
  Fp12 f = fp12_one();
  int e = 0;
  const uint64_t X = BLS_X_ABS;
  for (int bit = 62; bit >= 0; --bit) {
    if (bit != 62) f = sqr12(f);
    const int adds = (int)((X >> bit) & 1ull);
    for (int a = 0; a <= adds; ++a) {
      uint32_t g = 0;
#pragma unroll 1
      for (; g + 1 < n; g += 2) {
        Fp2 l0, l2, l3, m0, m2, m3;
        load_line(L, stride, k0 + g, e, l0, l2, l3);
        load_line(L, stride, k0 + g + 1, e, m0, m2, m3);
        f = fp12_mul_line2(f, l0, l2, l3, m0, m2, m3);
      }
#pragma unroll 1
      for (; g < n; ++g) {
        Fp2 l0, l2, l3;
        load_line(L, stride, k0 + g, e, l0, l2, l3);
        f = mul_line12(f, l0, l2, l3);
      }
      ++e;
    }
  }
  return fp12_conj(f);
}


}

template <int W>
__global__ __launch_bounds__(BLS_BLOCK) __attribute__((amdgpu_waves_per_eu(W, W))) void k_mlq(
    PipeBufs b, uint32_t first, uint32_t count, uint32_t units_paired, uint32_t* L, uint32_t stride,
    const uint32_t* items) {
  const uint32_t k = blockIdx.x * BLS_BLOCK + threadIdx.x;
  if (k >= count) return;
  const uint32_t i = items ? items[k] : first + k;
  if (!ml_live(b, i, units_paired)) return;
  const Fp* ch = b.chain + (size_t)CHAIN_WORDS * i;
  G1J rp;
  rp.x = ch[CH_RP + 0];
  rp.y = ch[CH_RP + 1];
  rp.z = ch[CH_RP + 2];
  const G1Eval P = g1_eval_affine_from_jac(rp);
  G2A q;
  q.x = Fp2{ch[CH_HQ + 0], ch[CH_HQ + 1]};
  q.y = Fp2{ch[CH_HQ + 2], ch[CH_HQ + 3]};
  q.inf = false;
  G2Proj T;
  T.x = q.x;
  T.y = q.y;
  T.z = fp2_one();
  Fp2 c0, c1, c2;
  int e = 0;
  const uint64_t X = BLS_X_ABS;
  for (int bit = 62; bit >= 0; --bit) {
    miller_dbl_step(T, c0, c1, c2);
    store_line(L, stride, k, e++, P, c0, c1, c2);
    if ((X >> bit) & 1ull) {
      miller_add_step(T, q, c0, c1, c2);
      store_line(L, stride, k, e++, P, c0, c1, c2);
    }
  }
}

template <int W>
__global__ __launch_bounds__(BLS_BLOCK) __attribute__((amdgpu_waves_per_eu(W, W))) void k_mlf(
    PipeBufs b, uint32_t first, uint32_t count, uint32_t units_paired, const uint32_t* L, uint32_t stride,
    const uint32_t* items, uint32_t per_lane) {
  const uint32_t k0 = per_lane * (blockIdx.x * BLS_BLOCK + threadIdx.x);
  if (k0 >= count) return;
  const uint32_t n = min(per_lane, count - k0);
  const uint32_t i0 = items ? items[k0] : first + k0;
  bool share = n > 1 && units_paired && b.ml_dom && !items && ml_live(b, i0, units_paired);
  for (uint32_t g = 1; share && g < n; ++g) {
    const uint32_t i = first + k0 + g;
    share = ml_live(b, i, units_paired) && i < b.indiv_vbase && b.ml_dom[i] == b.ml_dom[i0];
  }
  if (share) {
    b.f[i0] = ml_f(L, stride, k0, n);
    for (uint32_t g = 1; g < n; ++g) b.f[first + k0 + g] = fp12_one();
    return;
  }
  for (uint32_t g = 0; g < n; ++g) {
    const uint32_t i = items ? items[k0 + g] : first + k0 + g;
    if (ml_live(b, i, units_paired)) b.f[i] = ml_f(L, stride, k0 + g, 1);
  }
}

__device__ __forceinline__ uint32_t pair_swap(uint32_t v) {
  return (uint32_t)__builtin_amdgcn_mov_dpp((int)v, 0xB1, 0xF, 0xF, false);
}
__device__ __forceinline__ Fp pair_swap(const Fp& a) {
  Fp r;
#pragma unroll
  for (int w = 0; w < 12; ++w) r.l[w] = pair_swap(a.l[w]);
  return r;
}
__device__ __forceinline__ Fp2 pair_swap(const Fp2& a) { return Fp2{pair_swap(a.c0), pair_swap(a.c1)}; }
__device__ __forceinline__ Fp6 pair_swap(const Fp6& a) { return Fp6{pair_swap(a.c0), pair_swap(a.c1), pair_swap(a.c2)}; }

__device__ __forceinline__ Fp12 sqr12_pair(const Fp12& a, bool h) {
  const Fp6 m = fp12_sqr_half_prod(a, h);
  return fp12_sqr_half_join(m, pair_swap(m), h);
}

__device__ __forceinline__ Fp12 mul_line12_pair(const Fp12& f, const Fp2& l0, const Fp2& l2, const Fp2& l3, bool h) {
  const LineHalf own = fp12_line_half_prod(f, l0, l2, l3, h);
  return fp12_line_half_join(own, pair_swap(own.m), pair_swap(own.p), h);
}


template <int W>
__global__ __launch_bounds__(BLS_BLOCK) __attribute__((amdgpu_waves_per_eu(W, W))) void k_mlf2(
    PipeBufs b, uint32_t first, uint32_t count, uint32_t units_paired, const uint32_t* L, uint32_t stride,
    const uint32_t* items) {
  const uint32_t t = blockIdx.x * BLS_BLOCK + threadIdx.x;
  const uint32_t k = t >> 1;
  const bool h = (t & 1u) != 0u;
  if (k >= count) return;
  const uint32_t i = items ? items[k] : first + k;
  if (!ml_live(b, i, units_paired)) return;
  Fp12 f = fp12_one();
  int e = 0;
  const uint64_t X = BLS_X_ABS;
  for (int bit = 62; bit >= 0; --bit) {
    if (bit != 62) f = sqr12_pair(f, h);
    const int adds = (int)((X >> bit) & 1ull);
    for (int a = 0; a <= adds; ++a) {
      Fp2 l0, l2, l3;
      load_line(L, stride, k, e, l0, l2, l3);
      f = mul_line12_pair(f, l0, l2, l3, h);
      ++e;
    }
  }
  if (!h) b.f[i] = fp12_conj(f);
}

size_t mlq_line_words(uint32_t count) {
  const size_t stride = ((size_t)count + BLS_BLOCK - 1) / BLS_BLOCK * BLS_BLOCK;
  return stride * ML_EVENTS * LINE_WORDS;
}

hipError_t launch_k_mlqf(const PipeBufs& b, uint32_t first, uint32_t count, bool own_only, uint32_t* lines,
                         hipStream_t s, const uint32_t* items) {
  if (count == 0) return hipSuccess;
  const uint32_t stride = (count + BLS_BLOCK - 1) / BLS_BLOCK * BLS_BLOCK;
  const uint32_t up = (own_only || items) ? 0u : 1u;
  k_mlq<1><<<bls_grid_for(count), BLS_BLOCK, 0, s>>>(b, first, count, up, lines, stride, items);
  const uint32_t per_lane = b.mlf_pl ? b.mlf_pl : mlf_per_lane();
  if (per_lane == MLF_PAIR) {
    static const int w2 = [] {
      const char* e = getenv("BLS_MLF2_WAVES");
      return e && atoi(e) == 1 ? 1 : 2;
    }();
    if (w2 == 2) k_mlf2<2><<<bls_grid_for(2 * count), BLS_BLOCK, 0, s>>>(b, first, count, up, lines, stride, items);
    else k_mlf2<1><<<bls_grid_for(2 * count), BLS_BLOCK, 0, s>>>(b, first, count, up, lines, stride, items);
    return hipGetLastError();
  }
  const uint32_t lanes = (count + per_lane - 1) / per_lane;
  k_mlf<1><<<bls_grid_for(lanes), BLS_BLOCK, 0, s>>>(b, first, count, up, lines, stride, items, per_lane);
  return hipGetLastError();
}

uint32_t mlf_per_lane_fixed() {
  static const uint32_t fixed = [] {
    const char* e = getenv("BLS_MLF_PER_LANE");
    const int v = e ? atoi(e) : 0;
    return (v == 1 || v == 2 || v == 4 || v == (int)MLF_PAIR) ? (uint32_t)v : 0u;
  }();
  return fixed;
}

uint64_t mlf_pair_max() {
  static const uint64_t pair_max = [] {
    const char* e = getenv("BLS_MLF_PAIR_MAX");
    return e ? (uint64_t)strtoull(e, nullptr, 10) : 16384ull;
  }();
  return pair_max;
}

uint32_t mlf_per_lane_alone(uint32_t count) {
  static const bool off = [] {
    const char* e = getenv("BLS_MLF_ALONE");
    return e && atoi(e) == 0;
  }();
  if (off) return 0u;
  const uint32_t fixed = mlf_per_lane_fixed();
  if (fixed) return fixed;
  return count <= mlf_pair_max() ? MLF_PAIR : 1u;
}

uint32_t mlf_per_lane() {
  const uint32_t fixed = mlf_per_lane_fixed();
  const uint64_t pair_max = mlf_pair_max();
  static const uint64_t pl2_min = [] {
    const char* e = getenv("BLS_MLF_PL2_MIN");
    return e ? (uint64_t)strtoull(e, nullptr, 10) : 98304ull;
  }();
  static const uint64_t pl4_min = [] {
    const char* e = getenv("BLS_MLF_PL4_MIN");
    return e ? (uint64_t)strtoull(e, nullptr, 10) : 200000ull;
  }();
  if (fixed) return fixed;
  const uint64_t k = bls_sets_in_flight();
  return k > pl4_min ? 4u : (k > pl2_min ? 2u : (k > pair_max ? 1u : MLF_PAIR));
}
```

Measured before the change: 3.922 million sets/s.

## Add fused Fp2 mul/sqr primitive with row-form d28 MACs for chain and Miller-loop kernels

Adds a new Fp2 multiply and square primitive built on row-wise 28-bit digit multiply-accumulate inline assembly, using v_mad_u64_u32 and v_mad_i64_i32. It folds the Karatsuba-style combination into a single accumulator with signed rows, so each Fp2 product needs only two reductions instead of three separate Fp multiplications. The primitive is a noinline function that takes one operand through an LDS slot to cut register pressure at the call boundary. It is enabled in k_chain and k_mlq and adds test ops and a host build helper. The risks are the extra LDS traffic, call overhead, and a hard requirement that BLS_BLOCK equal one wavefront.

After: 4.196 million sets/s (median of 6 runs). +7.0%, better.

```diff
diff --git a/lodestar_amd/build.py b/lodestar_amd/build.py
--- a/lodestar_amd/build.py
+++ b/lodestar_amd/build.py
@@ -209,6 +209,22 @@
     return out
 
 
+def build_fp2_rows_host(verbose: bool = True) -> Path:
+    src = ROOT / "tests" / "native" / "fp2_rows_host.cpp"
+    out = ROOT / "tests" / "native" / "libfp2_rows_host.so"
+    key = hashlib.sha256(_headers_digest().encode() + src.read_bytes()).hexdigest()[:16]
+    stamp = out.with_suffix(".stamp")
+    if out.exists() and stamp.exists() and stamp.read_text() == key:
+        return out
+    cmd = ["g++", "-O2", "-std=c++17", "-shared", "-fPIC", "-I", str(CSRC), "-I", str(ROOT / "include"), "-o",
+           str(out), str(src)]
+    if verbose:
+        print("[build]", " ".join(cmd), flush=True)
+    subprocess.run(cmd, check=True)
+    stamp.write_text(key)
+    return out
+
+
 def build_smsum_host(verbose: bool = True, out: Path | None = None, extra: list[str] | None = None) -> Path:
     src = ROOT / "tests" / "native" / "smsum_host.cpp"
     out = out or ROOT / "tests" / "native" / "smsum_host"
diff --git a/lodestar_amd/csrc/bls/d28_rows.hpp b/lodestar_amd/csrc/bls/d28_rows.hpp
--- /dev/null
+++ b/lodestar_amd/csrc/bls/d28_rows.hpp
@@ -0,0 +1,481 @@
+#pragma once
+
+namespace bls {
+
+#if defined(__HIP_DEVICE_COMPILE__)
+__device__ __forceinline__ void d28_row_u1_asm(uint64_t* t, uint32_t a, const uint32_t* b) {
+  asm volatile("v_mad_u64_u32 %0, vcc, %1, %2, %0"
+               : "+v"(t[0])
+               : "v"(a), "v"(b[0])
+               : "vcc");
+}
+__device__ __forceinline__ void d28_row_s1_asm(uint64_t* t, uint32_t a, const uint32_t* b) {
+  asm volatile("v_mad_i64_i32 %0, vcc, %1, %2, %0"
+               : "+v"(t[0])
+               : "v"(a), "v"(b[0])
+               : "vcc");
+}
+__device__ __forceinline__ void d28_row_u2_asm(uint64_t* t, uint32_t a, const uint32_t* b) {
+  asm volatile("v_mad_u64_u32 %0, vcc, %2, %3, %0\n\t"
+               "v_mad_u64_u32 %1, vcc, %2, %4, %1"
+               : "+v"(t[0]), "+v"(t[1])
+               : "v"(a), "v"(b[0]), "v"(b[1])
+               : "vcc");
+}
+__device__ __forceinline__ void d28_row_s2_asm(uint64_t* t, uint32_t a, const uint32_t* b) {
+  asm volatile("v_mad_i64_i32 %0, vcc, %2, %3, %0\n\t"
+               "v_mad_i64_i32 %1, vcc, %2, %4, %1"
+               : "+v"(t[0]), "+v"(t[1])
+               : "v"(a), "v"(b[0]), "v"(b[1])
+               : "vcc");
+}
+__device__ __forceinline__ void d28_row_u3_asm(uint64_t* t, uint32_t a, const uint32_t* b) {
+  asm volatile("v_mad_u64_u32 %0, vcc, %3, %4, %0\n\t"
+               "v_mad_u64_u32 %1, vcc, %3, %5, %1\n\t"
+               "v_mad_u64_u32 %2, vcc, %3, %6, %2"
+               : "+v"(t[0]), "+v"(t[1]), "+v"(t[2])
+               : "v"(a), "v"(b[0]), "v"(b[1]), "v"(b[2])
+               : "vcc");
+}
+__device__ __forceinline__ void d28_row_s3_asm(uint64_t* t, uint32_t a, const uint32_t* b) {
+  asm volatile("v_mad_i64_i32 %0, vcc, %3, %4, %0\n\t"
+               "v_mad_i64_i32 %1, vcc, %3, %5, %1\n\t"
+               "v_mad_i64_i32 %2, vcc, %3, %6, %2"
+               : "+v"(t[0]), "+v"(t[1]), "+v"(t[2])
+               : "v"(a), "v"(b[0]), "v"(b[1]), "v"(b[2])
+               : "vcc");
+}
+__device__ __forceinline__ void d28_row_u4_asm(uint64_t* t, uint32_t a, const uint32_t* b) {
+  asm volatile("v_mad_u64_u32 %0, vcc, %4, %5, %0\n\t"
+               "v_mad_u64_u32 %1, vcc, %4, %6, %1\n\t"
+               "v_mad_u64_u32 %2, vcc, %4, %7, %2\n\t"
+               "v_mad_u64_u32 %3, vcc, %4, %8, %3"
+               : "+v"(t[0]), "+v"(t[1]), "+v"(t[2]), "+v"(t[3])
+               : "v"(a), "v"(b[0]), "v"(b[1]), "v"(b[2]), "v"(b[3])
+               : "vcc");
+}
+__device__ __forceinline__ void d28_row_s4_asm(uint64_t* t, uint32_t a, const uint32_t* b) {
+  asm volatile("v_mad_i64_i32 %0, vcc, %4, %5, %0\n\t"
+               "v_mad_i64_i32 %1, vcc, %4, %6, %1\n\t"
+               "v_mad_i64_i32 %2, vcc, %4, %7, %2\n\t"
+               "v_mad_i64_i32 %3, vcc, %4, %8, %3"
+               : "+v"(t[0]), "+v"(t[1]), "+v"(t[2]), "+v"(t[3])
+               : "v"(a), "v"(b[0]), "v"(b[1]), "v"(b[2]), "v"(b[3])
+               : "vcc");
+}
+__device__ __forceinline__ void d28_row_u5_asm(uint64_t* t, uint32_t a, const uint32_t* b) {
+  asm volatile("v_mad_u64_u32 %0, vcc, %5, %6, %0\n\t"
+               "v_mad_u64_u32 %1, vcc, %5, %7, %1\n\t"
+               "v_mad_u64_u32 %2, vcc, %5, %8, %2\n\t"
+               "v_mad_u64_u32 %3, vcc, %5, %9, %3\n\t"
+               "v_mad_u64_u32 %4, vcc, %5, %10, %4"
+               : "+v"(t[0]), "+v"(t[1]), "+v"(t[2]), "+v"(t[3]), "+v"(t[4])
+               : "v"(a), "v"(b[0]), "v"(b[1]), "v"(b[2]), "v"(b[3]), "v"(b[4])
+               : "vcc");
+}
+__device__ __forceinline__ void d28_row_s5_asm(uint64_t* t, uint32_t a, const uint32_t* b) {
+  asm volatile("v_mad_i64_i32 %0, vcc, %5, %6, %0\n\t"
+               "v_mad_i64_i32 %1, vcc, %5, %7, %1\n\t"
+               "v_mad_i64_i32 %2, vcc, %5, %8, %2\n\t"
+               "v_mad_i64_i32 %3, vcc, %5, %9, %3\n\t"
+               "v_mad_i64_i32 %4, vcc, %5, %10, %4"
+               : "+v"(t[0]), "+v"(t[1]), "+v"(t[2]), "+v"(t[3]), "+v"(t[4])
+               : "v"(a), "v"(b[0]), "v"(b[1]), "v"(b[2]), "v"(b[3]), "v"(b[4])
+               : "vcc");
+}
+__device__ __forceinline__ void d28_row_u6_asm(uint64_t* t, uint32_t a, const uint32_t* b) {
+  asm volatile("v_mad_u64_u32 %0, vcc, %6, %7, %0\n\t"
+               "v_mad_u64_u32 %1, vcc, %6, %8, %1\n\t"
+               "v_mad_u64_u32 %2, vcc, %6, %9, %2\n\t"
+               "v_mad_u64_u32 %3, vcc, %6, %10, %3\n\t"
+               "v_mad_u64_u32 %4, vcc, %6, %11, %4\n\t"
+               "v_mad_u64_u32 %5, vcc, %6, %12, %5"
+               : "+v"(t[0]), "+v"(t[1]), "+v"(t[2]), "+v"(t[3]), "+v"(t[4]), "+v"(t[5])
+               : "v"(a), "v"(b[0]), "v"(b[1]), "v"(b[2]), "v"(b[3]), "v"(b[4]), "v"(b[5])
+               : "vcc");
+}
+__device__ __forceinline__ void d28_row_s6_asm(uint64_t* t, uint32_t a, const uint32_t* b) {
+  asm volatile("v_mad_i64_i32 %0, vcc, %6, %7, %0\n\t"
+               "v_mad_i64_i32 %1, vcc, %6, %8, %1\n\t"
+               "v_mad_i64_i32 %2, vcc, %6, %9, %2\n\t"
+               "v_mad_i64_i32 %3, vcc, %6, %10, %3\n\t"
+               "v_mad_i64_i32 %4, vcc, %6, %11, %4\n\t"
+               "v_mad_i64_i32 %5, vcc, %6, %12, %5"
+               : "+v"(t[0]), "+v"(t[1]), "+v"(t[2]), "+v"(t[3]), "+v"(t[4]), "+v"(t[5])
+               : "v"(a), "v"(b[0]), "v"(b[1]), "v"(b[2]), "v"(b[3]), "v"(b[4]), "v"(b[5])
+               : "vcc");
+}
+__device__ __forceinline__ void d28_row_u7_asm(uint64_t* t, uint32_t a, const uint32_t* b) {
+  asm volatile("v_mad_u64_u32 %0, vcc, %7, %8, %0\n\t"
+               "v_mad_u64_u32 %1, vcc, %7, %9, %1\n\t"
+               "v_mad_u64_u32 %2, vcc, %7, %10, %2\n\t"
+               "v_mad_u64_u32 %3, vcc, %7, %11, %3\n\t"
+               "v_mad_u64_u32 %4, vcc, %7, %12, %4\n\t"
+               "v_mad_u64_u32 %5, vcc, %7, %13, %5\n\t"
+               "v_mad_u64_u32 %6, vcc, %7, %14, %6"
+               : "+v"(t[0]), "+v"(t[1]), "+v"(t[2]), "+v"(t[3]), "+v"(t[4]), "+v"(t[5]), "+v"(t[6])
+               : "v"(a), "v"(b[0]), "v"(b[1]), "v"(b[2]), "v"(b[3]), "v"(b[4]), "v"(b[5]), "v"(b[6])
+               : "vcc");
+}
+__device__ __forceinline__ void d28_row_s7_asm(uint64_t* t, uint32_t a, const uint32_t* b) {
+  asm volatile("v_mad_i64_i32 %0, vcc, %7, %8, %0\n\t"
+               "v_mad_i64_i32 %1, vcc, %7, %9, %1\n\t"
+               "v_mad_i64_i32 %2, vcc, %7, %10, %2\n\t"
+               "v_mad_i64_i32 %3, vcc, %7, %11, %3\n\t"
+               "v_mad_i64_i32 %4, vcc, %7, %12, %4\n\t"
+               "v_mad_i64_i32 %5, vcc, %7, %13, %5\n\t"
+               "v_mad_i64_i32 %6, vcc, %7, %14, %6"
+               : "+v"(t[0]), "+v"(t[1]), "+v"(t[2]), "+v"(t[3]), "+v"(t[4]), "+v"(t[5]), "+v"(t[6])
+               : "v"(a), "v"(b[0]), "v"(b[1]), "v"(b[2]), "v"(b[3]), "v"(b[4]), "v"(b[5]), "v"(b[6])
+               : "vcc");
+}
+__device__ __forceinline__ void d28_row_u8_asm(uint64_t* t, uint32_t a, const uint32_t* b) {
+  asm volatile("v_mad_u64_u32 %0, vcc, %8, %9, %0\n\t"
+               "v_mad_u64_u32 %1, vcc, %8, %10, %1\n\t"
+               "v_mad_u64_u32 %2, vcc, %8, %11, %2\n\t"
+               "v_mad_u64_u32 %3, vcc, %8, %12, %3\n\t"
+               "v_mad_u64_u32 %4, vcc, %8, %13, %4\n\t"
+               "v_mad_u64_u32 %5, vcc, %8, %14, %5\n\t"
+               "v_mad_u64_u32 %6, vcc, %8, %15, %6\n\t"
+               "v_mad_u64_u32 %7, vcc, %8, %16, %7"
+               : "+v"(t[0]), "+v"(t[1]), "+v"(t[2]), "+v"(t[3]), "+v"(t[4]), "+v"(t[5]), "+v"(t[6]), "+v"(t[7])
+               : "v"(a), "v"(b[0]), "v"(b[1]), "v"(b[2]), "v"(b[3]), "v"(b[4]), "v"(b[5]), "v"(b[6]), "v"(b[7])
+               : "vcc");
+}
+__device__ __forceinline__ void d28_row_s8_asm(uint64_t* t, uint32_t a, const uint32_t* b) {
+  asm volatile("v_mad_i64_i32 %0, vcc, %8, %9, %0\n\t"
+               "v_mad_i64_i32 %1, vcc, %8, %10, %1\n\t"
+               "v_mad_i64_i32 %2, vcc, %8, %11, %2\n\t"
+               "v_mad_i64_i32 %3, vcc, %8, %12, %3\n\t"
+               "v_mad_i64_i32 %4, vcc, %8, %13, %4\n\t"
+               "v_mad_i64_i32 %5, vcc, %8, %14, %5\n\t"
+               "v_mad_i64_i32 %6, vcc, %8, %15, %6\n\t"
+               "v_mad_i64_i32 %7, vcc, %8, %16, %7"
+               : "+v"(t[0]), "+v"(t[1]), "+v"(t[2]), "+v"(t[3]), "+v"(t[4]), "+v"(t[5]), "+v"(t[6]), "+v"(t[7])
+               : "v"(a), "v"(b[0]), "v"(b[1]), "v"(b[2]), "v"(b[3]), "v"(b[4]), "v"(b[5]), "v"(b[6]), "v"(b[7])
+               : "vcc");
+}
+__device__ __forceinline__ void d28_row_u9_asm(uint64_t* t, uint32_t a, const uint32_t* b) {
+  asm volatile("v_mad_u64_u32 %0, vcc, %9, %10, %0\n\t"
+               "v_mad_u64_u32 %1, vcc, %9, %11, %1\n\t"
+               "v_mad_u64_u32 %2, vcc, %9, %12, %2\n\t"
+               "v_mad_u64_u32 %3, vcc, %9, %13, %3\n\t"
+               "v_mad_u64_u32 %4, vcc, %9, %14, %4\n\t"
+               "v_mad_u64_u32 %5, vcc, %9, %15, %5\n\t"
+               "v_mad_u64_u32 %6, vcc, %9, %16, %6\n\t"
+               "v_mad_u64_u32 %7, vcc, %9, %17, %7\n\t"
+               "v_mad_u64_u32 %8, vcc, %9, %18, %8"
+               : "+v"(t[0]), "+v"(t[1]), "+v"(t[2]), "+v"(t[3]), "+v"(t[4]), "+v"(t[5]), "+v"(t[6]), "+v"(t[7]), "+v"(t[8])
+               : "v"(a), "v"(b[0]), "v"(b[1]), "v"(b[2]), "v"(b[3]), "v"(b[4]), "v"(b[5]), "v"(b[6]), "v"(b[7]), "v"(b[8])
+               : "vcc");
+}
+__device__ __forceinline__ void d28_row_s9_asm(uint64_t* t, uint32_t a, const uint32_t* b) {
+  asm volatile("v_mad_i64_i32 %0, vcc, %9, %10, %0\n\t"
+               "v_mad_i64_i32 %1, vcc, %9, %11, %1\n\t"
+               "v_mad_i64_i32 %2, vcc, %9, %12, %2\n\t"
+               "v_mad_i64_i32 %3, vcc, %9, %13, %3\n\t"
+               "v_mad_i64_i32 %4, vcc, %9, %14, %4\n\t"
+               "v_mad_i64_i32 %5, vcc, %9, %15, %5\n\t"
+               "v_mad_i64_i32 %6, vcc, %9, %16, %6\n\t"
+               "v_mad_i64_i32 %7, vcc, %9, %17, %7\n\t"
+               "v_mad_i64_i32 %8, vcc, %9, %18, %8"
+               : "+v"(t[0]), "+v"(t[1]), "+v"(t[2]), "+v"(t[3]), "+v"(t[4]), "+v"(t[5]), "+v"(t[6]), "+v"(t[7]), "+v"(t[8])
+               : "v"(a), "v"(b[0]), "v"(b[1]), "v"(b[2]), "v"(b[3]), "v"(b[4]), "v"(b[5]), "v"(b[6]), "v"(b[7]), "v"(b[8])
+               : "vcc");
+}
+__device__ __forceinline__ void d28_row_u10_asm(uint64_t* t, uint32_t a, const uint32_t* b) {
+  asm volatile("v_mad_u64_u32 %0, vcc, %10, %11, %0\n\t"
+               "v_mad_u64_u32 %1, vcc, %10, %12, %1\n\t"
+               "v_mad_u64_u32 %2, vcc, %10, %13, %2\n\t"
+               "v_mad_u64_u32 %3, vcc, %10, %14, %3\n\t"
+               "v_mad_u64_u32 %4, vcc, %10, %15, %4\n\t"
+               "v_mad_u64_u32 %5, vcc, %10, %16, %5\n\t"
+               "v_mad_u64_u32 %6, vcc, %10, %17, %6\n\t"
+               "v_mad_u64_u32 %7, vcc, %10, %18, %7\n\t"
+               "v_mad_u64_u32 %8, vcc, %10, %19, %8\n\t"
+               "v_mad_u64_u32 %9, vcc, %10, %20, %9"
+               : "+v"(t[0]), "+v"(t[1]), "+v"(t[2]), "+v"(t[3]), "+v"(t[4]), "+v"(t[5]), "+v"(t[6]), "+v"(t[7]), "+v"(t[8]), "+v"(t[9])
+               : "v"(a), "v"(b[0]), "v"(b[1]), "v"(b[2]), "v"(b[3]), "v"(b[4]), "v"(b[5]), "v"(b[6]), "v"(b[7]), "v"(b[8]), "v"(b[9])
+               : "vcc");
+}
+__device__ __forceinline__ void d28_row_s10_asm(uint64_t* t, uint32_t a, const uint32_t* b) {
+  asm volatile("v_mad_i64_i32 %0, vcc, %10, %11, %0\n\t"
+               "v_mad_i64_i32 %1, vcc, %10, %12, %1\n\t"
+               "v_mad_i64_i32 %2, vcc, %10, %13, %2\n\t"
+               "v_mad_i64_i32 %3, vcc, %10, %14, %3\n\t"
+               "v_mad_i64_i32 %4, vcc, %10, %15, %4\n\t"
+               "v_mad_i64_i32 %5, vcc, %10, %16, %5\n\t"
+               "v_mad_i64_i32 %6, vcc, %10, %17, %6\n\t"
+               "v_mad_i64_i32 %7, vcc, %10, %18, %7\n\t"
+               "v_mad_i64_i32 %8, vcc, %10, %19, %8\n\t"
+               "v_mad_i64_i32 %9, vcc, %10, %20, %9"
+               : "+v"(t[0]), "+v"(t[1]), "+v"(t[2]), "+v"(t[3]), "+v"(t[4]), "+v"(t[5]), "+v"(t[6]), "+v"(t[7]), "+v"(t[8]), "+v"(t[9])
+               : "v"(a), "v"(b[0]), "v"(b[1]), "v"(b[2]), "v"(b[3]), "v"(b[4]), "v"(b[5]), "v"(b[6]), "v"(b[7]), "v"(b[8]), "v"(b[9])
+               : "vcc");
+}
+__device__ __forceinline__ void d28_row_u11_asm(uint64_t* t, uint32_t a, const uint32_t* b) {
+  asm volatile("v_mad_u64_u32 %0, vcc, %11, %12, %0\n\t"
+               "v_mad_u64_u32 %1, vcc, %11, %13, %1\n\t"
+               "v_mad_u64_u32 %2, vcc, %11, %14, %2\n\t"
+               "v_mad_u64_u32 %3, vcc, %11, %15, %3\n\t"
+               "v_mad_u64_u32 %4, vcc, %11, %16, %4\n\t"
+               "v_mad_u64_u32 %5, vcc, %11, %17, %5\n\t"
+               "v_mad_u64_u32 %6, vcc, %11, %18, %6\n\t"
+               "v_mad_u64_u32 %7, vcc, %11, %19, %7\n\t"
+               "v_mad_u64_u32 %8, vcc, %11, %20, %8\n\t"
+               "v_mad_u64_u32 %9, vcc, %11, %21, %9\n\t"
+               "v_mad_u64_u32 %10, vcc, %11, %22, %10"
+               : "+v"(t[0]), "+v"(t[1]), "+v"(t[2]), "+v"(t[3]), "+v"(t[4]), "+v"(t[5]), "+v"(t[6]), "+v"(t[7]), "+v"(t[8]), "+v"(t[9]), "+v"(t[10])
+               : "v"(a), "v"(b[0]), "v"(b[1]), "v"(b[2]), "v"(b[3]), "v"(b[4]), "v"(b[5]), "v"(b[6]), "v"(b[7]), "v"(b[8]), "v"(b[9]), "v"(b[10])
+               : "vcc");
+}
+__device__ __forceinline__ void d28_row_s11_asm(uint64_t* t, uint32_t a, const uint32_t* b) {
+  asm volatile("v_mad_i64_i32 %0, vcc, %11, %12, %0\n\t"
+               "v_mad_i64_i32 %1, vcc, %11, %13, %1\n\t"
+               "v_mad_i64_i32 %2, vcc, %11, %14, %2\n\t"
+               "v_mad_i64_i32 %3, vcc, %11, %15, %3\n\t"
+               "v_mad_i64_i32 %4, vcc, %11, %16, %4\n\t"
+               "v_mad_i64_i32 %5, vcc, %11, %17, %5\n\t"
+               "v_mad_i64_i32 %6, vcc, %11, %18, %6\n\t"
+               "v_mad_i64_i32 %7, vcc, %11, %19, %7\n\t"
+               "v_mad_i64_i32 %8, vcc, %11, %20, %8\n\t"
+               "v_mad_i64_i32 %9, vcc, %11, %21, %9\n\t"
+               "v_mad_i64_i32 %10, vcc, %11, %22, %10"
+               : "+v"(t[0]), "+v"(t[1]), "+v"(t[2]), "+v"(t[3]), "+v"(t[4]), "+v"(t[5]), "+v"(t[6]), "+v"(t[7]), "+v"(t[8]), "+v"(t[9]), "+v"(t[10])
+               : "v"(a), "v"(b[0]), "v"(b[1]), "v"(b[2]), "v"(b[3]), "v"(b[4]), "v"(b[5]), "v"(b[6]), "v"(b[7]), "v"(b[8]), "v"(b[9]), "v"(b[10])
+               : "vcc");
+}
+__device__ __forceinline__ void d28_row_u12_asm(uint64_t* t, uint32_t a, const uint32_t* b) {
+  asm volatile("v_mad_u64_u32 %0, vcc, %12, %13, %0\n\t"
+               "v_mad_u64_u32 %1, vcc, %12, %14, %1\n\t"
+               "v_mad_u64_u32 %2, vcc, %12, %15, %2\n\t"
+               "v_mad_u64_u32 %3, vcc, %12, %16, %3\n\t"
+               "v_mad_u64_u32 %4, vcc, %12, %17, %4\n\t"
+               "v_mad_u64_u32 %5, vcc, %12, %18, %5\n\t"
+               "v_mad_u64_u32 %6, vcc, %12, %19, %6\n\t"
+               "v_mad_u64_u32 %7, vcc, %12, %20, %7\n\t"
+               "v_mad_u64_u32 %8, vcc, %12, %21, %8\n\t"
+               "v_mad_u64_u32 %9, vcc, %12, %22, %9\n\t"
+               "v_mad_u64_u32 %10, vcc, %12, %23, %10\n\t"
+               "v_mad_u64_u32 %11, vcc, %12, %24, %11"
+               : "+v"(t[0]), "+v"(t[1]), "+v"(t[2]), "+v"(t[3]), "+v"(t[4]), "+v"(t[5]), "+v"(t[6]), "+v"(t[7]), "+v"(t[8]), "+v"(t[9]), "+v"(t[10]), "+v"(t[11])
+               : "v"(a), "v"(b[0]), "v"(b[1]), "v"(b[2]), "v"(b[3]), "v"(b[4]), "v"(b[5]), "v"(b[6]), "v"(b[7]), "v"(b[8]), "v"(b[9]), "v"(b[10]), "v"(b[11])
+               : "vcc");
+}
+__device__ __forceinline__ void d28_row_s12_asm(uint64_t* t, uint32_t a, const uint32_t* b) {
+  asm volatile("v_mad_i64_i32 %0, vcc, %12, %13, %0\n\t"
+               "v_mad_i64_i32 %1, vcc, %12, %14, %1\n\t"
+               "v_mad_i64_i32 %2, vcc, %12, %15, %2\n\t"
+               "v_mad_i64_i32 %3, vcc, %12, %16, %3\n\t"
+               "v_mad_i64_i32 %4, vcc, %12, %17, %4\n\t"
+               "v_mad_i64_i32 %5, vcc, %12, %18, %5\n\t"
+               "v_mad_i64_i32 %6, vcc, %12, %19, %6\n\t"
+               "v_mad_i64_i32 %7, vcc, %12, %20, %7\n\t"
+               "v_mad_i64_i32 %8, vcc, %12, %21, %8\n\t"
+               "v_mad_i64_i32 %9, vcc, %12, %22, %9\n\t"
+               "v_mad_i64_i32 %10, vcc, %12, %23, %10\n\t"
+               "v_mad_i64_i32 %11, vcc, %12, %24, %11"
+               : "+v"(t[0]), "+v"(t[1]), "+v"(t[2]), "+v"(t[3]), "+v"(t[4]), "+v"(t[5]), "+v"(t[6]), "+v"(t[7]), "+v"(t[8]), "+v"(t[9]), "+v"(t[10]), "+v"(t[11])
+               : "v"(a), "v"(b[0]), "v"(b[1]), "v"(b[2]), "v"(b[3]), "v"(b[4]), "v"(b[5]), "v"(b[6]), "v"(b[7]), "v"(b[8]), "v"(b[9]), "v"(b[10]), "v"(b[11])
+               : "vcc");
+}
+__device__ __forceinline__ void d28_row_u13_asm(uint64_t* t, uint32_t a, const uint32_t* b) {
+  asm volatile("v_mad_u64_u32 %0, vcc, %13, %14, %0\n\t"
+               "v_mad_u64_u32 %1, vcc, %13, %15, %1\n\t"
+               "v_mad_u64_u32 %2, vcc, %13, %16, %2\n\t"
+               "v_mad_u64_u32 %3, vcc, %13, %17, %3\n\t"
+               "v_mad_u64_u32 %4, vcc, %13, %18, %4\n\t"
+               "v_mad_u64_u32 %5, vcc, %13, %19, %5\n\t"
+               "v_mad_u64_u32 %6, vcc, %13, %20, %6\n\t"
+               "v_mad_u64_u32 %7, vcc, %13, %21, %7\n\t"
+               "v_mad_u64_u32 %8, vcc, %13, %22, %8\n\t"
+               "v_mad_u64_u32 %9, vcc, %13, %23, %9\n\t"
+               "v_mad_u64_u32 %10, vcc, %13, %24, %10\n\t"
+               "v_mad_u64_u32 %11, vcc, %13, %25, %11\n\t"
+               "v_mad_u64_u32 %12, vcc, %13, %26, %12"
+               : "+v"(t[0]), "+v"(t[1]), "+v"(t[2]), "+v"(t[3]), "+v"(t[4]), "+v"(t[5]), "+v"(t[6]), "+v"(t[7]), "+v"(t[8]), "+v"(t[9]), "+v"(t[10]), "+v"(t[11]), "+v"(t[12])
+               : "v"(a), "v"(b[0]), "v"(b[1]), "v"(b[2]), "v"(b[3]), "v"(b[4]), "v"(b[5]), "v"(b[6]), "v"(b[7]), "v"(b[8]), "v"(b[9]), "v"(b[10]), "v"(b[11]), "v"(b[12])
+               : "vcc");
+}
+__device__ __forceinline__ void d28_row_s13_asm(uint64_t* t, uint32_t a, const uint32_t* b) {
+  asm volatile("v_mad_i64_i32 %0, vcc, %13, %14, %0\n\t"
+               "v_mad_i64_i32 %1, vcc, %13, %15, %1\n\t"
+               "v_mad_i64_i32 %2, vcc, %13, %16, %2\n\t"
+               "v_mad_i64_i32 %3, vcc, %13, %17, %3\n\t"
+               "v_mad_i64_i32 %4, vcc, %13, %18, %4\n\t"
+               "v_mad_i64_i32 %5, vcc, %13, %19, %5\n\t"
+               "v_mad_i64_i32 %6, vcc, %13, %20, %6\n\t"
+               "v_mad_i64_i32 %7, vcc, %13, %21, %7\n\t"
+               "v_mad_i64_i32 %8, vcc, %13, %22, %8\n\t"
+               "v_mad_i64_i32 %9, vcc, %13, %23, %9\n\t"
+               "v_mad_i64_i32 %10, vcc, %13, %24, %10\n\t"
+               "v_mad_i64_i32 %11, vcc, %13, %25, %11\n\t"
+               "v_mad_i64_i32 %12, vcc, %13, %26, %12"
+               : "+v"(t[0]), "+v"(t[1]), "+v"(t[2]), "+v"(t[3]), "+v"(t[4]), "+v"(t[5]), "+v"(t[6]), "+v"(t[7]), "+v"(t[8]), "+v"(t[9]), "+v"(t[10]), "+v"(t[11]), "+v"(t[12])
+               : "v"(a), "v"(b[0]), "v"(b[1]), "v"(b[2]), "v"(b[3]), "v"(b[4]), "v"(b[5]), "v"(b[6]), "v"(b[7]), "v"(b[8]), "v"(b[9]), "v"(b[10]), "v"(b[11]), "v"(b[12])
+               : "vcc");
+}
+__device__ __forceinline__ void d28_row_u14_asm(uint64_t* t, uint32_t a, const uint32_t* b) {
+  asm volatile("v_mad_u64_u32 %0, vcc, %14, %15, %0\n\t"
+               "v_mad_u64_u32 %1, vcc, %14, %16, %1\n\t"
+               "v_mad_u64_u32 %2, vcc, %14, %17, %2\n\t"
+               "v_mad_u64_u32 %3, vcc, %14, %18, %3\n\t"
+               "v_mad_u64_u32 %4, vcc, %14, %19, %4\n\t"
+               "v_mad_u64_u32 %5, vcc, %14, %20, %5\n\t"
+               "v_mad_u64_u32 %6, vcc, %14, %21, %6\n\t"
+               "v_mad_u64_u32 %7, vcc, %14, %22, %7\n\t"
+               "v_mad_u64_u32 %8, vcc, %14, %23, %8\n\t"
+               "v_mad_u64_u32 %9, vcc, %14, %24, %9\n\t"
+               "v_mad_u64_u32 %10, vcc, %14, %25, %10\n\t"
+               "v_mad_u64_u32 %11, vcc, %14, %26, %11\n\t"
+               "v_mad_u64_u32 %12, vcc, %14, %27, %12\n\t"
+               "v_mad_u64_u32 %13, vcc, %14, %28, %13"
+               : "+v"(t[0]), "+v"(t[1]), "+v"(t[2]), "+v"(t[3]), "+v"(t[4]), "+v"(t[5]), "+v"(t[6]), "+v"(t[7]), "+v"(t[8]), "+v"(t[9]), "+v"(t[10]), "+v"(t[11]), "+v"(t[12]), "+v"(t[13])
+               : "v"(a), "v"(b[0]), "v"(b[1]), "v"(b[2]), "v"(b[3]), "v"(b[4]), "v"(b[5]), "v"(b[6]), "v"(b[7]), "v"(b[8]), "v"(b[9]), "v"(b[10]), "v"(b[11]), "v"(b[12]), "v"(b[13])
+               : "vcc");
+}
+__device__ __forceinline__ void d28_row_s14_asm(uint64_t* t, uint32_t a, const uint32_t* b) {
+  asm volatile("v_mad_i64_i32 %0, vcc, %14, %15, %0\n\t"
+               "v_mad_i64_i32 %1, vcc, %14, %16, %1\n\t"
+               "v_mad_i64_i32 %2, vcc, %14, %17, %2\n\t"
+               "v_mad_i64_i32 %3, vcc, %14, %18, %3\n\t"
+               "v_mad_i64_i32 %4, vcc, %14, %19, %4\n\t"
+               "v_mad_i64_i32 %5, vcc, %14, %20, %5\n\t"
+               "v_mad_i64_i32 %6, vcc, %14, %21, %6\n\t"
+               "v_mad_i64_i32 %7, vcc, %14, %22, %7\n\t"
+               "v_mad_i64_i32 %8, vcc, %14, %23, %8\n\t"
+               "v_mad_i64_i32 %9, vcc, %14, %24, %9\n\t"
+               "v_mad_i64_i32 %10, vcc, %14, %25, %10\n\t"
+               "v_mad_i64_i32 %11, vcc, %14, %26, %11\n\t"
+               "v_mad_i64_i32 %12, vcc, %14, %27, %12\n\t"
+               "v_mad_i64_i32 %13, vcc, %14, %28, %13"
+               : "+v"(t[0]), "+v"(t[1]), "+v"(t[2]), "+v"(t[3]), "+v"(t[4]), "+v"(t[5]), "+v"(t[6]), "+v"(t[7]), "+v"(t[8]), "+v"(t[9]), "+v"(t[10]), "+v"(t[11]), "+v"(t[12]), "+v"(t[13])
+               : "v"(a), "v"(b[0]), "v"(b[1]), "v"(b[2]), "v"(b[3]), "v"(b[4]), "v"(b[5]), "v"(b[6]), "v"(b[7]), "v"(b[8]), "v"(b[9]), "v"(b[10]), "v"(b[11]), "v"(b[12]), "v"(b[13])
+               : "vcc");
+}
+__device__ __forceinline__ void d28_row_ux_asm(uint64_t* t, uint32_t a, const uint32_t* b) {
+  asm volatile("v_mad_u64_u32 %0, vcc, %14, %15, %0\n\t"
+               "v_mad_u64_u32 %1, vcc, %14, %16, %1\n\t"
+               "v_mad_u64_u32 %2, vcc, %14, %17, %2\n\t"
+               "v_mad_u64_u32 %3, vcc, %14, %18, %3\n\t"
+               "v_mad_u64_u32 %4, vcc, %14, %19, %4\n\t"
+               "v_mad_u64_u32 %5, vcc, %14, %20, %5\n\t"
+               "v_mad_u64_u32 %6, vcc, %14, %21, %6\n\t"
+               "v_mad_u64_u32 %7, vcc, %14, %22, %7\n\t"
+               "v_mad_u64_u32 %8, vcc, %14, %23, %8\n\t"
+               "v_mad_u64_u32 %9, vcc, %14, %24, %9\n\t"
+               "v_mad_u64_u32 %10, vcc, %14, %25, %10\n\t"
+               "v_mad_u64_u32 %11, vcc, %14, %26, %11\n\t"
+               "v_mad_u64_u32 %12, vcc, %14, %27, %12\n\t"
+               "v_mad_u64_u32 %13, vcc, %14, %28, 0"
+               : "+v"(t[0]), "+v"(t[1]), "+v"(t[2]), "+v"(t[3]), "+v"(t[4]), "+v"(t[5]), "+v"(t[6]), "+v"(t[7]), "+v"(t[8]), "+v"(t[9]), "+v"(t[10]), "+v"(t[11]), "+v"(t[12]), "=&v"(t[13])
+               : "v"(a), "v"(b[0]), "v"(b[1]), "v"(b[2]), "v"(b[3]), "v"(b[4]), "v"(b[5]), "v"(b[6]), "v"(b[7]), "v"(b[8]), "v"(b[9]), "v"(b[10]), "v"(b[11]), "v"(b[12]), "v"(b[13])
+               : "vcc");
+}
+__device__ __forceinline__ void d28_row_uz_asm(uint64_t* t, uint32_t a, const uint32_t* b) {
+  asm volatile("v_mad_u64_u32 %0, vcc, %14, %15, 0\n\t"
+               "v_mad_u64_u32 %1, vcc, %14, %16, 0\n\t"
+               "v_mad_u64_u32 %2, vcc, %14, %17, 0\n\t"
+               "v_mad_u64_u32 %3, vcc, %14, %18, 0\n\t"
+               "v_mad_u64_u32 %4, vcc, %14, %19, 0\n\t"
+               "v_mad_u64_u32 %5, vcc, %14, %20, 0\n\t"
+               "v_mad_u64_u32 %6, vcc, %14, %21, 0\n\t"
+               "v_mad_u64_u32 %7, vcc, %14, %22, 0\n\t"
+               "v_mad_u64_u32 %8, vcc, %14, %23, 0\n\t"
+               "v_mad_u64_u32 %9, vcc, %14, %24, 0\n\t"
+               "v_mad_u64_u32 %10, vcc, %14, %25, 0\n\t"
+               "v_mad_u64_u32 %11, vcc, %14, %26, 0\n\t"
+               "v_mad_u64_u32 %12, vcc, %14, %27, 0\n\t"
+               "v_mad_u64_u32 %13, vcc, %14, %28, 0"
+               : "=&v"(t[0]), "=&v"(t[1]), "=&v"(t[2]), "=&v"(t[3]), "=&v"(t[4]), "=&v"(t[5]), "=&v"(t[6]), "=&v"(t[7]), "=&v"(t[8]), "=&v"(t[9]), "=&v"(t[10]), "=&v"(t[11]), "=&v"(t[12]), "=&v"(t[13])
+               : "v"(a), "v"(b[0]), "v"(b[1]), "v"(b[2]), "v"(b[3]), "v"(b[4]), "v"(b[5]), "v"(b[6]), "v"(b[7]), "v"(b[8]), "v"(b[9]), "v"(b[10]), "v"(b[11]), "v"(b[12]), "v"(b[13])
+               : "vcc");
+}
+__device__ __forceinline__ void d28_row_p_asm(uint64_t* t, uint32_t m) {
+  asm volatile("v_mad_u64_u32 %0, vcc, %14, %15, %0\n\t"
+               "v_mad_u64_u32 %1, vcc, %14, %16, %1\n\t"
+               "v_mad_u64_u32 %2, vcc, %14, %17, %2\n\t"
+               "v_mad_u64_u32 %3, vcc, %14, %18, %3\n\t"
+               "v_mad_u64_u32 %4, vcc, %14, %19, %4\n\t"
+               "v_mad_u64_u32 %5, vcc, %14, %20, %5\n\t"
+               "v_mad_u64_u32 %6, vcc, %14, %21, %6\n\t"
+               "v_mad_u64_u32 %7, vcc, %14, %22, %7\n\t"
+               "v_mad_u64_u32 %8, vcc, %14, %23, %8\n\t"
+               "v_mad_u64_u32 %9, vcc, %14, %24, %9\n\t"
+               "v_mad_u64_u32 %10, vcc, %14, %25, %10\n\t"
+               "v_mad_u64_u32 %11, vcc, %14, %26, %11\n\t"
+               "v_mad_u64_u32 %12, vcc, %14, %27, %12\n\t"
+               "v_mad_u64_u32 %13, vcc, %14, %28, %13"
+               : "+v"(t[0]), "+v"(t[1]), "+v"(t[2]), "+v"(t[3]), "+v"(t[4]), "+v"(t[5]), "+v"(t[6]), "+v"(t[7]), "+v"(t[8]), "+v"(t[9]), "+v"(t[10]), "+v"(t[11]), "+v"(t[12]), "+v"(t[13])
+               : "v"(m), "s"(0xfffaaabu), "s"(0xfefffffu), "s"(0x3ffffb9u), "s"(0xfffeb15u), "s"(0x6241eabu), "s"(0xa0f6b0fu), "s"(0xf6730d2u), "s"(0xf38512bu), "s"(0x4774b84u), "s"(0x4bacd76u), "s"(0xba7b643u), "s"(0xe69a4b1u), "s"(0x1ea397fu), "s"(0x001a011u)
+               : "vcc");
+}
+#endif
+
+template <int N>
+BLS_HD void d28_row_u(uint64_t* t, uint32_t a, const uint32_t* b) {
+#if defined(__HIP_DEVICE_COMPILE__)
+  if constexpr (N == 1) d28_row_u1_asm(t, a, b);
+  else if constexpr (N == 2) d28_row_u2_asm(t, a, b);
+  else if constexpr (N == 3) d28_row_u3_asm(t, a, b);
+  else if constexpr (N == 4) d28_row_u4_asm(t, a, b);
+  else if constexpr (N == 5) d28_row_u5_asm(t, a, b);
+  else if constexpr (N == 6) d28_row_u6_asm(t, a, b);
+  else if constexpr (N == 7) d28_row_u7_asm(t, a, b);
+  else if constexpr (N == 8) d28_row_u8_asm(t, a, b);
+  else if constexpr (N == 9) d28_row_u9_asm(t, a, b);
+  else if constexpr (N == 10) d28_row_u10_asm(t, a, b);
+  else if constexpr (N == 11) d28_row_u11_asm(t, a, b);
+  else if constexpr (N == 12) d28_row_u12_asm(t, a, b);
+  else if constexpr (N == 13) d28_row_u13_asm(t, a, b);
+  else if constexpr (N == 14) d28_row_u14_asm(t, a, b);
+#else
+  for (int j = 0; j < N; ++j) t[j] += (uint64_t)a * b[j];
+#endif
+}
+template <int N>
+BLS_HD void d28_row_s(uint64_t* t, uint32_t a, const uint32_t* b) {
+#if defined(__HIP_DEVICE_COMPILE__)
+  if constexpr (N == 1) d28_row_s1_asm(t, a, b);
+  else if constexpr (N == 2) d28_row_s2_asm(t, a, b);
+  else if constexpr (N == 3) d28_row_s3_asm(t, a, b);
+  else if constexpr (N == 4) d28_row_s4_asm(t, a, b);
+  else if constexpr (N == 5) d28_row_s5_asm(t, a, b);
+  else if constexpr (N == 6) d28_row_s6_asm(t, a, b);
+  else if constexpr (N == 7) d28_row_s7_asm(t, a, b);
+  else if constexpr (N == 8) d28_row_s8_asm(t, a, b);
+  else if constexpr (N == 9) d28_row_s9_asm(t, a, b);
+  else if constexpr (N == 10) d28_row_s10_asm(t, a, b);
+  else if constexpr (N == 11) d28_row_s11_asm(t, a, b);
+  else if constexpr (N == 12) d28_row_s12_asm(t, a, b);
+  else if constexpr (N == 13) d28_row_s13_asm(t, a, b);
+  else if constexpr (N == 14) d28_row_s14_asm(t, a, b);
+#else
+  for (int j = 0; j < N; ++j) t[j] = (uint64_t)((int64_t)t[j] + (int64_t)(int32_t)a * (int64_t)(int32_t)b[j]);
+#endif
+}
+BLS_HD void d28_row_ux(uint64_t* t, uint32_t a, const uint32_t* b) {
+#if defined(__HIP_DEVICE_COMPILE__)
+  d28_row_ux_asm(t, a, b);
+#else
+  for (int j = 0; j < 13; ++j) t[j] += (uint64_t)a * b[j];
+  t[13] = (uint64_t)a * b[13];
+#endif
+}
+BLS_HD void d28_row_uz(uint64_t* t, uint32_t a, const uint32_t* b) {
+#if defined(__HIP_DEVICE_COMPILE__)
+  d28_row_uz_asm(t, a, b);
+#else
+  for (int j = 0; j < 14; ++j) t[j] = (uint64_t)a * b[j];
+#endif
+}
+BLS_HD void d28_row_p(uint64_t* t, uint32_t m) {
+#if defined(__HIP_DEVICE_COMPILE__)
+  d28_row_p_asm(t, m);
+#else
+  const uint32_t p[14] = {0xfffaaabu, 0xfefffffu, 0x3ffffb9u, 0xfffeb15u, 0x6241eabu, 0xa0f6b0fu, 0xf6730d2u, 0xf38512bu, 0x4774b84u, 0x4bacd76u, 0xba7b643u, 0xe69a4b1u, 0x1ea397fu, 0x001a011u};
+  for (int j = 0; j < 14; ++j) t[j] += (uint64_t)m * p[j];
+#endif
+}
+
+}
diff --git a/lodestar_amd/csrc/bls/field.hpp b/lodestar_amd/csrc/bls/field.hpp
--- a/lodestar_amd/csrc/bls/field.hpp
+++ b/lodestar_amd/csrc/bls/field.hpp
@@ -286,6 +286,7 @@
 }
 
 #define BLS_D28_MASK 0xFFFFFFFu
+#define BLS_FP2_SLOT_LANES 64
 #define BLS_NP28 0xFFCFFFDu
 BLS_HD uint32_t p28_digit(int k) {
   const uint32_t t[14] = {0xfffaaabu, 0xfefffffu, 0x3ffffb9u, 0xfffeb15u, 0x6241eabu, 0xa0f6b0fu, 0xf6730d2u,
@@ -499,6 +500,96 @@
   return Fp2{c0, fp_reduce_once(fp_redc_d28<true>(t))};
 }
 
+}
+#include "d28_rows.hpp"
+namespace bls {
+
+BLS_HD uint64_t c2w_col(int k) {
+  const uint64_t t[27] = {
+      0x00ffffffe5b6ffb1ull, 0x01ffffffc6cf1d19ull, 0x02ffffffa2f472d1ull, 0x03ffffff85b73e73ull, 0x04ffffff6407ca93ull,
+      0x05ffffff4ba3e8d0ull, 0x06ffffff2295b5e9ull, 0x07ffffff0215b241ull, 0x08fffffee90e10e7ull, 0x09fffffecd3726b3ull,
+      0x0afffffea44164a6ull, 0x0bfffffe81176f1dull, 0x0cfffffe6dd4425bull, 0x0c006802bff9cc2bull, 0x0b006802dff97fc7ull,
+      0x0a006802fff97fc6ull, 0x090068031ff97fc5ull, 0x080068033ff97fc4ull, 0x070068035ff97fc3ull, 0x060068037ff97fc2ull,
+      0x050068039ff97fc1ull, 0x04006803bff97fc0ull, 0x03006803dff97fbfull, 0x02006803fff97fbeull, 0x010068041ff97fbdull,
+      0x000068043ff97fbcull, 0x0000000a90dd0484ull};
+  return t[k];
+}
+
+BLS_HD Fp fp_redc_rows(uint64_t t[27]) {
+#pragma unroll
+  for (int i = 0; i < 13; ++i) {
+    const uint32_t m = ((uint32_t)t[i] * BLS_NP28) & BLS_D28_MASK;
+    d28_row_p(t + i, m);
+    t[i + 1] += t[i] >> 28;
+  }
+  d28_row_p(t + 13, ((uint32_t)t[13] * BLS_NP28) & 0xFFFFFu);
+  return fp_d28_tail(t);
+}
+
+BLS_HD void d28_rows_sum2(uint64_t t[27], const uint32_t x0[14], const uint32_t y0[14], const uint32_t x1[14],
+                          const uint32_t y1[14]) {
+  d28_row_uz(t, x0[0], y0);
+  d28_row_u<14>(t, x1[0], y1);
+#pragma unroll
+  for (int i = 1; i < 14; ++i) {
+    d28_row_ux(t + i, x0[i], y0);
+    d28_row_u<14>(t + i, x1[i], y1);
+  }
+}
+
+BLS_HD Fp2 fp2_mul_rows(const Fp& a0, const Fp& a1, const Fp& b0, const Fp& b1) {
+  uint32_t x0[14], x1[14], y0[14], y1[14], ny1[14];
+  fp_to_d28(a0, x0);
+  fp_to_d28(a1, x1);
+  fp_to_d28(b0, y0);
+  fp_to_d28(b1, y1);
+#pragma unroll
+  for (int j = 0; j < 14; ++j) ny1[j] = 0u - y1[j];
+  uint64_t t[27];
+#pragma unroll
+  for (int k = 0; k < 27; ++k) t[k] = c2w_col(k);
+#pragma unroll
+  for (int i = 0; i < 14; ++i) {
+    d28_row_u<14>(t + i, x0[i], y0);
+    d28_row_s<14>(t + i, x1[i], ny1);
+  }
+  const Fp c0 = fp_reduce_once(fp_redc_rows(t));
+  BLS_PIN_FP(c0);
+  BLS_SCHED_FENCE();
+  d28_rows_sum2(t, x0, y1, x1, y0);
+  return Fp2{c0, fp_reduce_once(fp_redc_rows(t))};
+}
+
+BLS_HD Fp2 fp2_sqr_rows(const Fp& a0, const Fp& a1) {
+  uint32_t x0[14], x1[14], d0[14], r0[14], r1[14];
+  fp_to_d28(a0, x0);
+  fp_to_d28(a1, x1);
+#pragma unroll
+  for (int j = 0; j < 14; ++j) {
+    d0[j] = x0[j] << 1;
+    r0[j] = d0[j];
+    r1[j] = 0u - (x1[j] << 1);
+  }
+  uint64_t t[27];
+#pragma unroll
+  for (int k = 0; k < 27; ++k) t[k] = c2w_col(k);
+#define BLS_SQR_ROW(i)                              \
+  r0[i] = x0[i];                                    \
+  r1[i] = 0u - x1[i];                               \
+  d28_row_u<14 - (i)>(t + 2 * (i), x0[i], r0 + (i)); \
+  d28_row_s<14 - (i)>(t + 2 * (i), x1[i], r1 + (i));
+  BLS_SQR_ROW(0) BLS_SQR_ROW(1) BLS_SQR_ROW(2) BLS_SQR_ROW(3) BLS_SQR_ROW(4) BLS_SQR_ROW(5) BLS_SQR_ROW(6)
+  BLS_SQR_ROW(7) BLS_SQR_ROW(8) BLS_SQR_ROW(9) BLS_SQR_ROW(10) BLS_SQR_ROW(11) BLS_SQR_ROW(12) BLS_SQR_ROW(13)
+#undef BLS_SQR_ROW
+  const Fp c0 = fp_reduce_once(fp_redc_rows(t));
+  BLS_PIN_FP(c0);
+  BLS_SCHED_FENCE();
+  d28_row_uz(t, d0[0], x1);
+#pragma unroll
+  for (int i = 1; i < 14; ++i) d28_row_ux(t + i, d0[i], x1);
+  return Fp2{c0, fp_reduce_once(fp_redc_rows(t))};
+}
+
 #if defined(__HIP_DEVICE_COMPILE__)
 __device__ __forceinline__ void bls_mac(uint64_t& lo, uint32_t& hi, uint32_t a, uint32_t b) {
   uint64_t cc;
@@ -649,6 +740,56 @@
 BLS_FP_MUL_ATTR Fp fp_mul_w(BLS_W12(a), BLS_W12(b)) { return fp_mul_inl(BLS_FP_OF(a), BLS_FP_OF(b)); }
 BLS_FP_MUL_ATTR Fp fp_sqr_w(BLS_W12(a)) { return fp_sqr_dev(BLS_FP_OF(a)); }
 __device__ __forceinline__ Fp fp_mul(const Fp& a, const Fp& b) { return fp_mul_w(BLS_L12(a), BLS_L12(b)); }
+#if defined(BLS_FP_D28)
+typedef __attribute__((address_space(3))) uint64_t* bls_fp2_slot_t;
+typedef uint32_t bls_w24 __attribute__((ext_vector_type(24)));
+__device__ __forceinline__ bls_w24 fp2_to_w24(const Fp2& a) {
+  bls_w24 r;
+#pragma unroll
+  for (int k = 0; k < 12; ++k) {
+    r[k] = a.c0.l[k];
+    r[12 + k] = a.c1.l[k];
+  }
+  return r;
+}
+__device__ __forceinline__ Fp2 fp2_of_w24(const bls_w24& v) {
+  Fp2 r;
+#pragma unroll
+  for (int k = 0; k < 12; ++k) {
+    r.c0.l[k] = v[k];
+    r.c1.l[k] = v[12 + k];
+  }
+  return r;
+}
+static __device__ __attribute__((noinline)) bls_w24 fp2_mul_w(BLS_W12(a), BLS_W12(c), bls_fp2_slot_t s) {
+  Fp b0, b1;
+#pragma unroll
+  for (int k = 0; k < 6; ++k) {
+    const uint64_t u = s[BLS_FP2_SLOT_LANES * k], v = s[BLS_FP2_SLOT_LANES * (6 + k)];
+    b0.l[2 * k] = (uint32_t)u;
+    b0.l[2 * k + 1] = (uint32_t)(u >> 32);
+    b1.l[2 * k] = (uint32_t)v;
+    b1.l[2 * k + 1] = (uint32_t)(v >> 32);
+  }
+  return fp2_to_w24(fp2_mul_rows(BLS_FP_OF(a), BLS_FP_OF(c), b0, b1));
+}
+static __device__ __attribute__((noinline)) bls_w24 fp2_sqr_w(BLS_W12(a), BLS_W12(c)) {
+  return fp2_to_w24(fp2_sqr_rows(BLS_FP_OF(a), BLS_FP_OF(c)));
+}
+__device__ __forceinline__ Fp2 fp2_mul_prim(const Fp2& a, const Fp2& b) {
+  __shared__ uint64_t slot[12 * BLS_FP2_SLOT_LANES];
+  const bls_fp2_slot_t s = (bls_fp2_slot_t)&slot[threadIdx.x];
+#pragma unroll
+  for (int k = 0; k < 6; ++k) {
+    s[BLS_FP2_SLOT_LANES * k] = ((uint64_t)b.c0.l[2 * k + 1] << 32) | b.c0.l[2 * k];
+    s[BLS_FP2_SLOT_LANES * (6 + k)] = ((uint64_t)b.c1.l[2 * k + 1] << 32) | b.c1.l[2 * k];
+  }
+  return fp2_of_w24(fp2_mul_w(BLS_L12(a.c0), BLS_L12(a.c1), s));
+}
+__device__ __forceinline__ Fp2 fp2_sqr_prim(const Fp2& a) {
+  return fp2_of_w24(fp2_sqr_w(BLS_L12(a.c0), BLS_L12(a.c1)));
+}
+#endif
 #else
 BLS_HD Fp fp_mul(const Fp& a, const Fp& b) {
   BLS_COUNT_FPM();
@@ -975,24 +1116,36 @@
 BLS_HD Fp2 fp2_mul_fp(const Fp2& a, const Fp& b) { return Fp2{fp_mul(a.c0, b), fp_mul(a.c1, b)}; }
 
 BLS_HD Fp2 fp2_mul(const Fp2& a, const Fp2& b) {
+#if defined(__HIP_DEVICE_COMPILE__) && defined(BLS_FP2_PRIM)
+  return fp2_mul_prim(a, b);
+#else
   Fp t0 = fp_mul(a.c0, b.c0);
   Fp t1 = fp_mul(a.c1, b.c1);
   Fp t2 = fp_mul(fp_add_nr(a.c0, a.c1), fp_add_nr(b.c0, b.c1));
   return Fp2{fp_sub(t0, t1), fp_sub(fp_sub(t2, t0), t1)};
+#endif
 }
 
 BLS_HD Fp2 fp2_mul_s(const Fp2& a, const Fp2& b) {
+#if defined(__HIP_DEVICE_COMPILE__) && defined(BLS_FP2_PRIM)
+  return fp2_mul_prim(a, b);
+#else
   Fp t0 = fp_mul(a.c0, b.c0);
   Fp t1 = fp_mul(a.c1, b.c1);
   Fp t2 = fp_mul(fp_reduce_2p(fp_add_nr(a.c0, a.c1)), fp_add_nr(b.c0, b.c1));
   return Fp2{fp_sub(t0, t1), fp_sub(fp_sub(t2, t0), t1)};
+#endif
 }
 BLS_HD Fp2 fp2_add_nr(const Fp2& a, const Fp2& b) { return Fp2{fp_add_nr(a.c0, b.c0), fp_add_nr(a.c1, b.c1)}; }
 
 BLS_HD Fp2 fp2_sqr(const Fp2& a) {
+#if defined(__HIP_DEVICE_COMPILE__) && defined(BLS_FP2_PRIM)
+  return fp2_sqr_prim(a);
+#else
   Fp t0 = fp_mul(fp_add_nr(a.c0, a.c1), fp_sub_nr(a.c0, a.c1));
   Fp t1 = fp_mul(fp_add_nr(a.c0, a.c0), a.c1);
   return Fp2{t0, t1};
+#endif
 }
 
 BLS_HD Fp2 fp2_mul_xi(const Fp2& a) { return Fp2{fp_sub(a.c0, a.c1), fp_add(a.c0, a.c1)}; }
diff --git a/lodestar_amd/csrc/kernels/field_ops.hpp b/lodestar_amd/csrc/kernels/field_ops.hpp
--- a/lodestar_amd/csrc/kernels/field_ops.hpp
+++ b/lodestar_amd/csrc/kernels/field_ops.hpp
@@ -2,6 +2,8 @@
 
 #include "../launchers.hpp"
 #include "../bls/selftest_ops.hpp"
+
+static_assert(BLS_BLOCK == 64, "one wavefront per block (the Fp2 primitive's LDS slot, FOP_FP2_*_W)");
 
 namespace bls {
 
@@ -35,6 +37,9 @@
   FOP_FP2_INV,
   FOP_FP2_SQRT,
   FOP_LIN8,
+  FOP_FP2_MUL_W,
+  FOP_FP2_SQR_W,
+  FOP_FP2_CHAIN_W,
   FOP_COUNT
 };
 #define FOP_D28_FLAG 0x100u
@@ -45,7 +50,9 @@
                  op == FOP_CANON3 || op == FOP_SQR || op == FOP_SQR_D28_LAZY || op == FOP_INV ||
                  op == FOP_INV_GCD || op == FOP_SQRT
              ? 12
-         : op == FOP_FP2_MUL_D28 || op == FOP_FP2_MUL || op == FOP_FP2_MUL_S || op == FOP_LZ_FP2_OPS ? 48
+         : op == FOP_FP2_MUL_D28 || op == FOP_FP2_MUL || op == FOP_FP2_MUL_S || op == FOP_LZ_FP2_OPS ||
+                 op == FOP_FP2_MUL_W || op == FOP_FP2_CHAIN_W
+             ? 48
          : op == FOP_LZ_MUL_RAW                                                                        ? 28
          : op == FOP_LZ_SQR_RAW                                                                        ? 14
          : op == FOP_LIN8                                                                              ? FOP_LIN8_IN
@@ -53,7 +60,8 @@
 }
 constexpr int field_op_out_words(uint32_t op) {
   return op == FOP_FP2_MUL_D28 || op == FOP_FP2_SQR_D28 || op == FOP_FP2_MUL || op == FOP_FP2_SQR ||
-                 op == FOP_FP2_MUL_S || op == FOP_FP2_INV
+                 op == FOP_FP2_MUL_S || op == FOP_FP2_INV || op == FOP_FP2_MUL_W || op == FOP_FP2_SQR_W ||
+                 op == FOP_FP2_CHAIN_W
              ? 24
          : op == FOP_LZ_MUL_RAW || op == FOP_LZ_SQR_RAW ? 14
          : op == FOP_LZ_FP_OPS                          ? 120
@@ -140,6 +148,17 @@
     y[0] = fp2_sqrt(fop_ld2(x, 0), r) ? 1u : 0u;
     fop_st2(y + 1, 0, r);
   }
+#if defined(__HIP_DEVICE_COMPILE__)
+  else if constexpr (OP == FOP_FP2_MUL_W) fop_st2(y, 0, fp2_mul_prim(fop_ld2(x, 0), fop_ld2(x, 1)));
+  else if constexpr (OP == FOP_FP2_SQR_W) fop_st2(y, 0, fp2_sqr_prim(fop_ld2(x, 0)));
+  else if constexpr (OP == FOP_FP2_CHAIN_W) {
+    const Fp2 a = fop_ld2(x, 0), b = fop_ld2(x, 1);
+    const Fp2 r1 = fp2_mul_prim(a, b);
+    const Fp2 r2 = fp2_mul_prim(r1, b);
+    const Fp2 r3 = fp2_mul_prim(b, r2);
+    fop_st2(y, 0, fp2_mul_prim(r3, r1));
+  }
+#endif
 #endif
 }
 
@@ -235,6 +254,9 @@
     FOP_CASE(FOP_SQRT);
     FOP_CASE(FOP_FP2_INV);
     FOP_CASE(FOP_FP2_SQRT);
+    FOP_CASE(FOP_FP2_MUL_W);
+    FOP_CASE(FOP_FP2_SQR_W);
+    FOP_CASE(FOP_FP2_CHAIN_W);
     case FOP_LIN8:
       k_field_lin8<true><<<bls_grid_for(n), BLS_BLOCK, 0, s>>>(in, n, out);
       break;
diff --git a/lodestar_amd/csrc/kernels/k_chain.hip b/lodestar_amd/csrc/kernels/k_chain.hip
--- a/lodestar_amd/csrc/kernels/k_chain.hip
+++ b/lodestar_amd/csrc/kernels/k_chain.hip
@@ -1,7 +1,10 @@
 #define BLS_FP_D28 1
+#define BLS_FP2_PRIM 1
 #include "../launchers.hpp"
 
 using namespace bls;
+
+static_assert(BLS_BLOCK == BLS_FP2_SLOT_LANES, "the Fp2 primitive's LDS slot holds one wavefront per block");
 
 namespace {
 
diff --git a/lodestar_amd/csrc/kernels/k_mlq.hip b/lodestar_amd/csrc/kernels/k_mlq.hip
--- a/lodestar_amd/csrc/kernels/k_mlq.hip
+++ b/lodestar_amd/csrc/kernels/k_mlq.hip
@@ -1,10 +1,13 @@
 #define BLS_FP_D28 1
+#define BLS_FP2_PRIM 1
 #include <stdlib.h>
 
 #include "../launchers.hpp"
 #include "bls/pairing.hpp"
 
 using namespace bls;
+
+static_assert(BLS_BLOCK == BLS_FP2_SLOT_LANES, "the Fp2 primitive's LDS slot holds one wavefront per block");
 
 namespace {
 
```
